# Shekhale/gbnns_dim_red

Hardware: AMD Instinct MI355X
Metric: queries/sec @ recall@1>=0.95, SIFT1M 128->32 (higher is better)
Workload: dtype f32

## Files before the change

### gbnns_dim_red_amd/csrc/walk_hot.hip

```cpp
#include "launch_util.h"
#include "walk_lists.h"

#ifndef GBNNS_HOT1_LB
#define GBNNS_HOT1_LB (GBNNS_HOT1_QLDS ? 8 : 7)
#endif
namespace gbnns {

namespace {


__device__ __forceinline__ bool reg1_select_slow(RegList<1>& L, uint64_t mu, int& tsize, uint64_t* tie, uint32_t worst,
                                                 uint64_t lmask, int lane, uint32_t& node) {
    int best = -1;
    uint32_t hi_p = 0;
    if (mu) {
        hi_p = readlane_u32(L.hi[0], __ffsll((unsigned long long)mu) - 1);
        const uint64_t ms = __ballot(!(L.lo[0] & 1u) && L.hi[0] == hi_p) & lmask;
        if (ms) best = 63 - __clzll((long long)ms);
    }
    if (tsize > 0 && (best < 0 || hi_p == worst)) {
        uint32_t v = (lane < tsize) ? key_id(tie[lane]) + 1u : 0u;
        int w = lane;
        int lane_here = lane;
        asm volatile("" : "+v"(lane_here));
#pragma unroll
        for (int off = 32; off > 0; off >>= 1) {
            const int partner = (lane_here ^ off) << 2;
            const uint32_t ov = (uint32_t)__builtin_amdgcn_ds_bpermute(partner, (int)v);
            const int ow = __builtin_amdgcn_ds_bpermute(partner, w);
            if (ov > v) { v = ov; w = ow; }
        }
        v = (uint32_t)__builtin_amdgcn_readfirstlane((int)v);
        w = __builtin_amdgcn_readfirstlane(w);
        const uint32_t lid = (best >= 0) ? (readlane_u32(L.lo[0], best) >> 1) : 0u;
        if (best < 0 || v - 1u > lid) {
            node = v - 1u;
            if (lane == 0) tie[w] = tie[tsize - 1];
            tsize -= 1;
            wave_sync();
            return true;
        }
    }
    if (best < 0) return false;
    node = readlane_u32(L.lo[0], best) >> 1;
    if (lane == best) L.lo[0] |= 1u;
    return true;
}

template <int R>
__device__ __forceinline__ bool regN_select_slow(RegList<R>& L, int p1, int& tsize, uint64_t* tie, uint32_t worst, int ef,
                                                 int lane, uint32_t& node) {
    int best = -1;
    uint32_t hi_p = 0;
    if (p1 >= 0) {
        hi_p = L.hi_at(p1);
#pragma unroll
        for (int r = 0; r < R; ++r) {
            const uint64_t ms = __ballot(!(L.lo[r] & 1u) && L.hi[r] == hi_p) & RegList<R>::lane_mask(r, ef);
            if (ms) best = r * 64 + 63 - __clzll((long long)ms);
        }
    }
    if (tsize > 0 && (best < 0 || hi_p == worst)) {
        uint32_t v = (lane < tsize) ? key_id(tie[lane]) + 1u : 0u;
        int w = lane;
        int lane_here = lane;
        asm volatile("" : "+v"(lane_here));
#pragma unroll
        for (int off = 32; off > 0; off >>= 1) {
            const int partner = (lane_here ^ off) << 2;
            const uint32_t ov = (uint32_t)__builtin_amdgcn_ds_bpermute(partner, (int)v);
            const int ow = __builtin_amdgcn_ds_bpermute(partner, w);
            if (ov > v) { v = ov; w = ow; }
        }
        v = (uint32_t)__builtin_amdgcn_readfirstlane((int)v);
        w = __builtin_amdgcn_readfirstlane(w);
        const uint32_t lid = (best >= 0) ? (L.lo_at(best) >> 1) : 0u;
        if (best < 0 || v - 1u > lid) {
            node = v - 1u;
            if (lane == 0) tie[w] = tie[tsize - 1];
            tsize -= 1;
            wave_sync();
            return true;
        }
    }
    if (best < 0) return false;
    node = L.lo_at(best) >> 1;
    L.mark_expanded(best, lane);
    return true;
}

#define GBNNS_VS_ASM(T0, T1, T2, ADDR)                                                                                                   \
        "s_bfe_u32 %[mulc], %[shr], 0x50008\n\t"                                    \
        "s_lshl_b32 %[mulc], 0x9E3779B1, %[mulc]\n\t"                                                                  \
        "v_mul_lo_u32 " T0 ", %[id], %[mulc]\n\t"                                                                       \
        "s_and_b32 exec_lo, exec_lo, 0x55555555\n\t"                                                                   \
        "s_and_b32 exec_hi, exec_hi, 0x55555555\n\t"                                                                   \
        "s_mov_b64 %[fresh], 0\n\t"                                                                                    \
        "s_cmp_lg_u32 %[shr], 0\n\t"                                                                                   \
        "v_mul_hi_u32 " T1 ", " T0 ", %[nb]\n\t"                                                                         \
        "v_lshl_add_u32 " ADDR ", " T1 ", 4, %[basev]\n\t"                                                               \
        "s_cbranch_scc1 4f\n"                                                                                          \
        "1:\n\t"                                                                                                       \
        "ds_read_b128 v[60:63], " ADDR "\n\t"                                                                           \
        "s_waitcnt lgkmcnt(0)\n\t"                                                                                     \
        "v_bfe_u32 v56, v60, 0, 24\n\t"                                                                    \
        "v_alignbit_b32 v57, v61, v60, 24\n\t"                            \
        "v_alignbit_b32 v58, v62, v61, 16\n\t"                                               \
        "v_lshrrev_b32 v59, 8, v62\n\t"                                                      \
        "v_bfe_u32 " T1 ", v63, 0, 24\n\t"                                                   \
        "v_bfe_u32 v57, v57, 0, 24\n\t"                                                                                \
        "v_bfe_u32 v58, v58, 0, 24\n\t"                                                                                \
        "v_xor_b32 v56, v56, %[id]\n\t"                                                                                \
        "v_xor_b32 v57, v57, %[id]\n\t"                                                                                \
        "v_xor_b32 v58, v58, %[id]\n\t"                                                                                \
        "v_xor_b32 v59, v59, %[id]\n\t"                                                                                \
        "v_xor_b32 " T1 ", " T1 ", %[id]\n\t"                                                                            \
        "v_min3_u32 v56, v56, v57, v58\n\t"                                                                            \
        "v_min3_u32 v56, v56, v59, " T1 "\n\t"                                           \
        "v_lshrrev_b32 " T1 ", 24, v63\n\t"                                                       \
        "v_cmp_ne_u32 vcc, 0, v56\n\t"                                                                                 \
        "s_and_b64 exec, exec, vcc\n\t"                                        \
        "s_cbranch_execz 9f\n\t"                                                                                       \
        "s_mov_b64 %[act], exec\n\t"                                                                                   \
        "v_cmp_gt_u32 vcc, 5, " T1 "\n\t"                                                                               \
        "s_and_b64 exec, exec, vcc\n\t"                                      \
        "s_cbranch_execz 3f\n\t"                                                                                       \
        "v_mov_b32 " T1 ", 0x1000000\n\t"                                                                               \
        "ds_add_rtn_u32 " T0 ", " ADDR ", " T1 " offset:12\n\t"                                   \
        "v_lshrrev_b32 " T2 ", 8, %[id]\n\t"                                                                            \
        "s_waitcnt lgkmcnt(0)\n\t"                                                                                     \
        "v_lshrrev_b32 " T0 ", 24, " T0 "\n\t"                                                                           \
        "v_cmp_gt_u32 vcc, 5, " T0 "\n\t"                                                                               \
        "s_and_b64 exec, exec, vcc\n\t"                                         \
        "s_cbranch_execz 3f\n\t"                                                                                       \
        "v_mad_u32_u24 " T0 ", " T0 ", 3, " ADDR "\n\t"                                     \
        "ds_write_b8 " T0 ", %[id]\n\t"                                                                                 \
        "ds_write_b8 " T0 ", " T2 " offset:1\n\t"                                                                        \
        "ds_write_b8_d16_hi " T0 ", %[id] offset:2\n\t"                                                                 \
        "s_or_b64 %[fresh], %[fresh], exec\n\t"                                                                        \
        "s_andn2_b64 %[act], %[act], exec\n"                                                                           \
        "3:\n\t"                                                                                                       \
        "s_mov_b64 exec, %[act]\n\t"                                    \
        "s_cbranch_execz 9f\n\t"                                                                                       \
        "v_add_u32 " ADDR ", 16, " ADDR "\n\t"                                                                           \
        "v_cmp_eq_u32 vcc, %[end], " ADDR "\n\t"                                                                        \
        "v_cndmask_b32 " ADDR ", " ADDR ", %[basev], vcc\n\t"                                                            \
        "s_branch 1b\n"                                                                                                \
        "4:\n\t"                                                                          \
        "s_lshl_b32 %[mulc], %[nb], 4\n\t"                                                                             \
        "v_mul_lo_u32 " T0 ", " T0 ", %[nb]\n\t"                               \
        "v_lshrrev_b32 " T0 ", %[shr], " T0 "\n\t"                                                           \
        "v_lshl_or_b32 " T2 ", " T0 ", 16, " T0 "\n"                          \
        "5:\n\t"                                                                                                       \
        "ds_read_b128 v[60:63], " ADDR "\n\t"                                                                           \
        "s_waitcnt lgkmcnt(0)\n\t"                                                                                     \
        "v_xor_b32 v56, v60, " T2 "\n\t"                                                                                \
        "v_xor_b32 v57, v61, " T2 "\n\t"                                                                                \
        "v_xor_b32 v58, v62, " T2 "\n\t"                                                                                \
        "v_xor_b32 v59, v63, " T2 "\n\t"                                                                                \
        "v_pk_min_u16 v56, v56, v57\n\t"                                                                               \
        "v_pk_min_u16 v58, v58, v59\n\t"                                                                               \
        "v_bfe_u32 " T1 ", v63, 16, 12\n\t"                                                       \
        "v_pk_min_u16 v56, v56, v58\n\t"                                                                               \
        "v_mad_u32_u16 v56, v56, v56, 0 op_sel:[0,1,0,0]\n\t"   \
        "v_cmp_ne_u32 vcc, 0, v56\n\t"                                                                                 \
        "s_and_b64 exec, exec, vcc\n\t"                                                                                \
        "s_cbranch_execz 9f\n\t"                                                                                       \
        "s_mov_b64 %[act], exec\n\t"                                                                                   \
        "v_cmp_gt_u32 vcc, 7, " T1 "\n\t"                                                                               \
        "s_and_b64 exec, exec, vcc\n\t"                                                                                \
        "s_cbranch_execz 6f\n\t"                                                                                       \
        "v_mov_b32 " T1 ", 0x10000\n\t"                                                                                 \
        "ds_add_rtn_u32 " T0 ", " ADDR ", " T1 " offset:12\n\t"                                                           \
        "s_waitcnt lgkmcnt(0)\n\t"                                                                                     \
        "v_bfe_u32 " T0 ", " T0 ", 16, 12\n\t"                                                                           \
        "v_cmp_gt_u32 vcc, 7, " T0 "\n\t"                                                                               \
        "s_and_b64 exec, exec, vcc\n\t"                                                                                \
        "s_cbranch_execz 6f\n\t"                                                                                       \
        "v_lshl_add_u32 " T0 ", " T0 ", 1, " ADDR "\n\t"                                                                  \
        "ds_write_b16 " T0 ", " T2 "\n\t"                                                                                \
        "s_or_b64 %[fresh], %[fresh], exec\n\t"                                                                        \
        "s_andn2_b64 %[act], %[act], exec\n"                                                                           \
        "6:\n\t"                                                                                                       \
        "s_mov_b64 exec, %[act]\n\t"                                                                                   \
        "s_cbranch_execz 9f\n\t"                                                                                       \
        "v_and_b32 " T0 ", 7, " T2 "\n\t"                         \
        "v_lshl_add_u32 " T0 ", " T0 ", 4, 16\n\t"                \
        "v_add_u32 " ADDR ", " ADDR ", " T0 "\n\t"                                                                        \
        "s_bfe_u32 vcc_lo, %[shr], 0x10010\n\t"                 \
        "s_lshl_b32 vcc_lo, 0x10001000, vcc_lo\n\t"                                                                    \
        "v_add_u32 " T2 ", vcc_lo, " T2 "\n\t"                                          \
        "v_cmp_le_u32 vcc, %[end], " ADDR "\n\t"                                                                        \
        "v_subrev_u32 " T0 ", %[mulc], " ADDR "\n\t"                       \
        "v_cndmask_b32 " ADDR ", " ADDR ", " T0 ", vcc\n\t"                                                               \
        "s_and_b32 vcc_lo, %[shr], 0xF0000000\n\t"            \
        "v_cmp_gt_u32 vcc, vcc_lo, " T2 "\n\t"                    \
        "s_andn2_b64 %[act], exec, vcc\n\t"                     \
        "s_lshl_b64 %[act], %[act], 1\n\t"                                                                             \
        "s_or_b64 %[fresh], %[fresh], %[act]\n\t"                                                                      \
        "s_and_b64 exec, exec, vcc\n\t"                                                                                \
        "s_cbranch_execnz 5b\n"                                                                                        \
        "9:\n\t"

#define GBNNS_L2_DIST_ASM(Q0A, Q0B, Q1A, Q1B, Q2A, Q2B, Q3A, Q3B, W1, W2, W3)                                                     \
        "s_waitcnt vmcnt(3)\n\t"                                \
        "v_pk_add_f32 v[40:41], v[40:41], " Q0A " neg_lo:[0,1] neg_hi:[0,1]\n\t"                                        \
        "v_pk_add_f32 v[42:43], v[42:43], " Q0B " neg_lo:[0,1] neg_hi:[0,1]\n\t"                                        \
        "v_pk_mul_f32 v[40:41], v[40:41], v[40:41]\n\t"                                                                \
        "v_pk_mul_f32 v[42:43], v[42:43], v[42:43]\n\t"                                                                \
        W1                                                                                                             \
        "v_pk_add_f32 v[44:45], v[44:45], " Q1A " neg_lo:[0,1] neg_hi:[0,1]\n\t"                                        \
        "v_pk_add_f32 v[46:47], v[46:47], " Q1B " neg_lo:[0,1] neg_hi:[0,1]\n\t"                                        \
        "v_pk_mul_f32 v[44:45], v[44:45], v[44:45]\n\t"                                                                \
        "v_pk_mul_f32 v[46:47], v[46:47], v[46:47]\n\t"                                                                \
        W2                                                                                                             \
        "v_pk_add_f32 v[48:49], v[48:49], " Q2A " neg_lo:[0,1] neg_hi:[0,1]\n\t"                                        \
        "v_pk_add_f32 v[50:51], v[50:51], " Q2B " neg_lo:[0,1] neg_hi:[0,1]\n\t"                                        \
        "v_pk_mul_f32 v[48:49], v[48:49], v[48:49]\n\t"                                                                \
        "v_pk_mul_f32 v[50:51], v[50:51], v[50:51]\n\t"                                                                \
        W3                                                                                                             \
        "v_pk_add_f32 v[52:53], v[52:53], " Q3A " neg_lo:[0,1] neg_hi:[0,1]\n\t"                                        \
        "v_pk_add_f32 v[54:55], v[54:55], " Q3B " neg_lo:[0,1] neg_hi:[0,1]\n\t"                                        \
        "v_pk_mul_f32 v[52:53], v[52:53], v[52:53]\n\t"                                                                \
        "v_pk_mul_f32 v[54:55], v[54:55], v[54:55]\n\t"                                                                \
        "v_pk_add_f32 v[60:61], v[40:41], v[44:45]\n\t"                                     \
        "v_pk_add_f32 v[62:63], v[42:43], v[46:47]\n\t"                                                                \
        "v_pk_add_f32 v[60:61], v[60:61], v[48:49]\n\t"                                                                \
        "v_pk_add_f32 v[62:63], v[62:63], v[50:51]\n\t"                                                                \
        "v_pk_add_f32 v[60:61], v[60:61], v[52:53]\n\t"                                                                \
        "v_pk_add_f32 v[62:63], v[62:63], v[54:55]\n\t"                                                                \
        "s_nop 1\n\t"                                                                                                  \
        "v_mov_b32_dpp v56, v60 quad_perm:[0,0,2,2] row_mask:0xf bank_mask:0xf\n\t"                                    \
        "v_mov_b32_dpp v57, v61 quad_perm:[0,0,2,2] row_mask:0xf bank_mask:0xf\n\t"                                    \
        "v_mov_b32_dpp v58, v62 quad_perm:[0,0,2,2] row_mask:0xf bank_mask:0xf\n\t"                                    \
        "v_mov_b32_dpp v59, v63 quad_perm:[0,0,2,2] row_mask:0xf bank_mask:0xf\n\t"                                    \
        "v_pk_add_f32 v[56:57], v[56:57], v[40:41]\n\t"                               \
        "v_pk_add_f32 v[58:59], v[58:59], v[42:43]\n\t"                                                                \
        "v_pk_add_f32 v[56:57], v[56:57], v[44:45]\n\t"                                                                \
        "v_pk_add_f32 v[58:59], v[58:59], v[46:47]\n\t"                                                                \
        "v_pk_add_f32 v[56:57], v[56:57], v[48:49]\n\t"                                                                \
        "v_pk_add_f32 v[58:59], v[58:59], v[50:51]\n\t"                                                                \
        "v_pk_add_f32 v[56:57], v[56:57], v[52:53]\n\t"                                                                \
        "v_pk_add_f32 v[58:59], v[58:59], v[54:55]\n\t"                                                                \
        "v_add_f32 %[key], v56, v57\n\t"                                                                               \
        "v_add_f32 %[key], %[key], v58\n\t"                                                                            \
        "v_add_f32 %[key], %[key], v59\n\t"                                                                            \
        "v_or_b32 %[key], 0x80000000, %[key]"

#define GBNNS_DOT_DIST_ASM(Q0A, Q0B, Q1A, Q1B, Q2A, Q2B, Q3A, Q3B, W1, W2, W3)                                                    \
        "s_waitcnt vmcnt(3)\n\t"                                                                                       \
        "v_pk_mul_f32 v[40:41], v[40:41], " Q0A "\n\t"                                                                 \
        "v_pk_mul_f32 v[42:43], v[42:43], " Q0B "\n\t"                                                                 \
        W1                                                                                                             \
        "v_pk_mul_f32 v[44:45], v[44:45], " Q1A "\n\t"                                                                 \
        "v_pk_mul_f32 v[46:47], v[46:47], " Q1B "\n\t"                                                                 \
        W2                                                                                                             \
        "v_pk_mul_f32 v[48:49], v[48:49], " Q2A "\n\t"                                                                 \
        "v_pk_mul_f32 v[50:51], v[50:51], " Q2B "\n\t"                                                                 \
        W3                                                                                                             \
        "v_pk_mul_f32 v[52:53], v[52:53], " Q3A "\n\t"                                                                 \
        "v_pk_mul_f32 v[54:55], v[54:55], " Q3B "\n\t"                                                                 \
        "v_mov_b32 v56, 0\n\t"                                     \
        "v_mov_b32 v57, 0\n\t"                                                                                         \
        "v_pk_add_f32 v[60:61], v[56:57], v[40:41]\n\t"           \
        "v_pk_add_f32 v[62:63], v[56:57], v[42:43]\n\t"                                                                \
        "v_pk_add_f32 v[60:61], v[60:61], v[44:45]\n\t"                                                                \
        "v_pk_add_f32 v[62:63], v[62:63], v[46:47]\n\t"                                                                \
        "v_pk_add_f32 v[60:61], v[60:61], v[48:49]\n\t"                                                                \
        "v_pk_add_f32 v[62:63], v[62:63], v[50:51]\n\t"                                                                \
        "v_pk_add_f32 v[60:61], v[60:61], v[52:53]\n\t"                                                                \
        "v_pk_add_f32 v[62:63], v[62:63], v[54:55]\n\t"                                                                \
        "s_nop 1\n\t"                                                                                                  \
        "v_mov_b32_dpp v56, v60 quad_perm:[0,0,2,2] row_mask:0xf bank_mask:0xf\n\t"      \
        "v_mov_b32_dpp v57, v61 quad_perm:[0,0,2,2] row_mask:0xf bank_mask:0xf\n\t"                                    \
        "v_mov_b32_dpp v58, v62 quad_perm:[0,0,2,2] row_mask:0xf bank_mask:0xf\n\t"                                    \
        "v_mov_b32_dpp v59, v63 quad_perm:[0,0,2,2] row_mask:0xf bank_mask:0xf\n\t"                                    \
        "v_pk_add_f32 v[56:57], v[60:61], v[56:57]\n\t"                             \
        "v_pk_add_f32 v[58:59], v[62:63], v[58:59]\n\t"                                                                \
        "v_add_f32 %[key], v56, v57\n\t"                                                    \
        "v_add_f32 v60, v58, v59\n\t"                                               \
        "v_add_f32 %[key], %[key], v60\n\t"                                                                            \
        "v_xor_b32 %[key], 0x80000000, %[key]\n\t"                                       \
        "v_add_f32 %[key], 0, %[key]\n\t"                                                         \
        "v_ashrrev_i32 v60, 31, %[key]\n\t"                     \
        "v_or_b32 v60, 0x80000000, v60\n\t"                                                                            \
        "v_xor_b32 %[key], %[key], v60"

#define GBNNS_LOADS_SPEC(O1, O2, O3)                                    \
        "global_load_dwordx4 v[40:43], %[roff], %[db]\n\t"              \
        "global_load_dwordx4 v[44:47], %[roff], %[db] offset:" O1 "\n\t" \
        "global_load_dwordx4 v[48:51], %[roff], %[db] offset:" O2 "\n\t" \
        "global_load_dwordx4 v[52:55], %[roff], %[db] offset:" O3 "\n\t"
#define GBNNS_LOADS_TESTED(O1, O2, O3)                                                                                 \
        "s_lshr_b64 %[act], %[fresh], 1\n\t"                             \
        "s_or_b64 exec, %[act], %[fresh]\n\t"                                                                          \
        "s_and_b32 exec_lo, exec_lo, 0x55555555\n\t"                                     \
        "s_and_b32 exec_hi, exec_hi, 0x55555555\n\t"                                                                   \
        "s_lshl_b64 %[act], exec, 1\n\t"                                                                               \
        "s_or_b64 exec, exec, %[act]\n\t"                                              \
        "s_cbranch_execz 8f\n\t"                                                                                       \
        GBNNS_LOADS_SPEC(O1, O2, O3)                                                                                   \
        "s_mov_b64 exec, %[sv]\n\t"
#define GBNNS_LOADS_DYN_BEFORE(O1, O2, O3)      \
        "s_cmp_eq_u32 %[spec], 0\n\t"           \
        "s_cbranch_scc1 12f\n\t"                \
        GBNNS_LOADS_SPEC(O1, O2, O3)            \
        "12:\n\t"
#define GBNNS_LOADS_DYN_AFTER(O1, O2, O3)       \
        "s_cmp_lg_u32 %[spec], 0\n\t"           \
        "s_cbranch_scc0 10f\n\t"                \
        "s_mov_b64 exec, %[sv]\n\t"             \
        "s_branch 11f\n"                        \
        "10:\n\t"                               \
        GBNNS_LOADS_TESTED(O1, O2, O3)          \
        "11:\n\t"
#define GBNNS_HOT_END "\n8:\n\ts_mov_b64 exec, %[sv]"

#define GBNNS_HOT_CLOBBERS_40                                                                                           \
    "vcc", "scc", "memory", "v40", "v41", "v42", "v43", "v44", "v45", "v46", "v47", "v48", "v49", "v50", "v51", "v52", "v53", "v54",  \
        "v55", "v56", "v57", "v58", "v59", "v60", "v61", "v62", "v63"

template <int METRIC = 0, bool QLDS = false, bool SPEC = !QLDS, bool DYN = false, typename QP>
__device__ __forceinline__ uint32_t hot_expand(const char* db_base, uint32_t roff, uint32_t nb, uint64_t valid, uint32_t lds_base,
                                               uint32_t nbuckets, QP qh, uint32_t qaddr, uint64_t& claimed, uint32_t shr, uint64_t& overflowed,
                                               uint32_t spec = 0u) {
    const uint32_t end = lds_base + (nbuckets << 4);
    uint32_t basev = lds_base, key, mulc;
    uint64_t fresh, act, sv;
#define GBNNS_Q(T) [qa##T] "v"(f32x2{qh[T].x, qh[T].y}), [qb##T] "v"(f32x2{qh[T].z, qh[T].w})
#define GBNNS_HOT_OUT [fresh] "=&s"(fresh), [act] "=&s"(act), [sv] "=&s"(sv), [mulc] "=&s"(mulc), [key] "=&v"(key)
#define GBNNS_HOT_IN [id] "v"(nb), [valid] "s"(valid), [end] "s"(end), [basev] "v"(basev), [shr] "s"(shr), [nb] "s"(nbuckets), \
                     [roff] "v"(roff), [db] "s"(db_base)
#define GBNNS_HOT_IN_QREG GBNNS_HOT_IN, GBNNS_Q(0), GBNNS_Q(1), GBNNS_Q(2), GBNNS_Q(3)
#define GBNNS_HOT_IN_QLDS GBNNS_HOT_IN, [qaddr] "v"(qaddr)
#define GBNNS_HOT_IN_QLDS_DYN GBNNS_HOT_IN_QLDS, [spec] "s"(spec)
#define GBNNS_HOT_OUT_QREG GBNNS_HOT_OUT, [t0] "=&v"(t0), [t1] "=&v"(t1), [t2] "=&v"(t2), [addr] "=&v"(addr)
#define GBNNS_HOT_OUT_QLDS GBNNS_HOT_OUT
#define GBNNS_VS_QREG GBNNS_VS_ASM("%[t0]", "%[t1]", "%[t2]", "%[addr]")
#define GBNNS_VS_QLDS GBNNS_VS_ASM("v36", "v37", "v38", "v39")
#define GBNNS_CLOB_QREG GBNNS_HOT_CLOBBERS_40
#define GBNNS_CLOB_QLDS "v36", "v37", "v38", "v39", GBNNS_HOT_CLOBBERS_40
#define GBNNS_HOT_STMT(LOADS_BEFORE, VS, AFTER_VS, DIST, OUTS, OPS, CLOB)                      \
    asm volatile("s_mov_b64 %[sv], exec\n\t"                                                   \
                 "s_mov_b64 exec, %[valid]\n\t" LOADS_BEFORE VS AFTER_VS DIST GBNNS_HOT_END      \
                 : OUTS                                                                        \
                 : OPS                                                                         \
                 : CLOB)
#define GBNNS_RESTORE_EXEC "s_mov_b64 exec, %[sv]\n\t"
#define GBNNS_L2_QREG                                                                                                          \
    GBNNS_L2_DIST_ASM("%[qa0]", "%[qb0]", "%[qa1]", "%[qb1]", "%[qa2]", "%[qb2]", "%[qa3]", "%[qb3]", "s_waitcnt vmcnt(2)\n\t", \
                      "s_waitcnt vmcnt(1)\n\t", "s_waitcnt vmcnt(0)\n\t")
#define GBNNS_L2_QLDS                                                                                                          \
    "ds_read_b128 v[36:39], %[qaddr]\n\t"                       \
    "ds_read_b128 v[56:59], %[qaddr] offset:16\n\t"           \
    "ds_read_b128 v[60:63], %[qaddr] offset:32\n\t"                                                                           \
    "s_waitcnt lgkmcnt(2)\n\t"                                                                                                \
    GBNNS_L2_DIST_ASM("v[36:37]", "v[38:39]", "v[56:57]", "v[58:59]", "v[60:61]", "v[62:63]", "v[36:37]", "v[38:39]",          \
                      "ds_read_b128 v[36:39], %[qaddr] offset:48\n\ts_waitcnt vmcnt(2) lgkmcnt(2)\n\t",                        \
                      "s_waitcnt vmcnt(1) lgkmcnt(1)\n\t", "s_waitcnt vmcnt(0) lgkmcnt(0)\n\t")
#define GBNNS_DOT_QREG                                                                                                          \
    GBNNS_DOT_DIST_ASM("%[qa0]", "%[qb0]", "%[qa1]", "%[qb1]", "%[qa2]", "%[qb2]", "%[qa3]", "%[qb3]", "s_waitcnt vmcnt(2)\n\t", \
                       "s_waitcnt vmcnt(1)\n\t", "s_waitcnt vmcnt(0)\n\t")
#define GBNNS_DOT_QLDS                                                                                                         \
    "ds_read_b128 v[36:39], %[qaddr]\n\t"                                                                                     \
    "ds_read_b128 v[56:59], %[qaddr] offset:32\n\t"                                                                           \
    "ds_read_b128 v[60:63], %[qaddr] offset:64\n\t"                                                                           \
    "s_waitcnt lgkmcnt(2)\n\t"                                                                                                \
    GBNNS_DOT_DIST_ASM("v[36:37]", "v[38:39]", "v[56:57]", "v[58:59]", "v[60:61]", "v[62:63]", "v[36:37]", "v[38:39]",         \
                       "ds_read_b128 v[36:39], %[qaddr] offset:96\n\ts_waitcnt vmcnt(2) lgkmcnt(2)\n\t",                       \
                       "s_waitcnt vmcnt(1) lgkmcnt(1)\n\t", "s_waitcnt vmcnt(0) lgkmcnt(0)\n\t")
    uint32_t t0, t1, t2, addr;
    (void)t0; (void)t1; (void)t2; (void)addr;
    if constexpr (DYN) {
        static_assert(!DYN || QLDS, "the dynamic order exists for the query-in-LDS instances");
        if constexpr (METRIC == 0) GBNNS_HOT_STMT(GBNNS_LOADS_DYN_BEFORE("16", "32", "48"), GBNNS_VS_QLDS, GBNNS_LOADS_DYN_AFTER("16", "32", "48"), GBNNS_L2_QLDS, GBNNS_HOT_OUT_QLDS, GBNNS_HOT_IN_QLDS_DYN, GBNNS_CLOB_QLDS);
        else GBNNS_HOT_STMT(GBNNS_LOADS_DYN_BEFORE("32", "64", "96"), GBNNS_VS_QLDS, GBNNS_LOADS_DYN_AFTER("32", "64", "96"), GBNNS_DOT_QLDS, GBNNS_HOT_OUT_QLDS, GBNNS_HOT_IN_QLDS_DYN, GBNNS_CLOB_QLDS);
    } else if constexpr (METRIC == 0) {
        if constexpr (!QLDS && SPEC) GBNNS_HOT_STMT(GBNNS_LOADS_SPEC("16", "32", "48"), GBNNS_VS_QREG, GBNNS_RESTORE_EXEC, GBNNS_L2_QREG, GBNNS_HOT_OUT_QREG, GBNNS_HOT_IN_QREG, GBNNS_CLOB_QREG);
        else if constexpr (!QLDS) GBNNS_HOT_STMT("", GBNNS_VS_QREG, GBNNS_LOADS_TESTED("16", "32", "48"), GBNNS_L2_QREG, GBNNS_HOT_OUT_QREG, GBNNS_HOT_IN_QREG, GBNNS_CLOB_QREG);
        else if constexpr (SPEC) GBNNS_HOT_STMT(GBNNS_LOADS_SPEC("16", "32", "48"), GBNNS_VS_QLDS, GBNNS_RESTORE_EXEC, GBNNS_L2_QLDS, GBNNS_HOT_OUT_QLDS, GBNNS_HOT_IN_QLDS, GBNNS_CLOB_QLDS);
        else GBNNS_HOT_STMT("", GBNNS_VS_QLDS, GBNNS_LOADS_TESTED("16", "32", "48"), GBNNS_L2_QLDS, GBNNS_HOT_OUT_QLDS, GBNNS_HOT_IN_QLDS, GBNNS_CLOB_QLDS);
    } else {
        if constexpr (!QLDS && SPEC) GBNNS_HOT_STMT(GBNNS_LOADS_SPEC("32", "64", "96"), GBNNS_VS_QREG, GBNNS_RESTORE_EXEC, GBNNS_DOT_QREG, GBNNS_HOT_OUT_QREG, GBNNS_HOT_IN_QREG, GBNNS_CLOB_QREG);
        else if constexpr (!QLDS) GBNNS_HOT_STMT("", GBNNS_VS_QREG, GBNNS_LOADS_TESTED("32", "64", "96"), GBNNS_DOT_QREG, GBNNS_HOT_OUT_QREG, GBNNS_HOT_IN_QREG, GBNNS_CLOB_QREG);
        else if constexpr (SPEC) GBNNS_HOT_STMT(GBNNS_LOADS_SPEC("32", "64", "96"), GBNNS_VS_QLDS, GBNNS_RESTORE_EXEC, GBNNS_DOT_QLDS, GBNNS_HOT_OUT_QLDS, GBNNS_HOT_IN_QLDS, GBNNS_CLOB_QLDS);
        else GBNNS_HOT_STMT("", GBNNS_VS_QLDS, GBNNS_LOADS_TESTED("32", "64", "96"), GBNNS_DOT_QLDS, GBNNS_HOT_OUT_QLDS, GBNNS_HOT_IN_QLDS, GBNNS_CLOB_QLDS);
    }
#undef GBNNS_HOT_STMT
#undef GBNNS_HOT_IN_QREG
#undef GBNNS_HOT_IN_QLDS
#undef GBNNS_HOT_IN_QLDS_DYN
#undef GBNNS_CLOB_QLDS
#undef GBNNS_CLOB_QREG
#undef GBNNS_VS_QLDS
#undef GBNNS_VS_QREG
#undef GBNNS_HOT_OUT_QLDS
#undef GBNNS_HOT_OUT_QREG
#undef GBNNS_Q
#undef GBNNS_HOT_OUT
#undef GBNNS_HOT_IN
    claimed = fresh & 0x5555555555555555ull;
    overflowed = fresh & 0xAAAAAAAAAAAAAAAAull;
    return key;
}

template <int R, bool WIDE = false, int METRIC = 0, bool SPEC1 = GBNNS_HOT1_SPEC != 0>
__device__ __forceinline__ void walk_hot_one(const WalkParams& p, uint32_t qi, unsigned char* smem) {
    const int lane = lane_id();
    const uint32_t slot = (uint32_t)lane >> 1, half = (uint32_t)lane & 1u;
    const int ef = p.ef;
#ifdef GBNNS_LIFE_STAMPS
    const unsigned long long life0 = __builtin_amdgcn_s_memrealtime();
#endif
    constexpr bool QLDS = R == 1 && GBNNS_HOT1_QLDS, SPEC = R == 1 ? SPEC1 : true;
    uint64_t* tie = reinterpret_cast<uint64_t*>(smem);
    uint64_t* stage = tie + kRegTieCap;
    float* qf = reinterpret_cast<float*>(QLDS ? stage + reg_stage_slots(R) : stage);
    uint32_t* hash = reinterpret_cast<uint32_t*>(stage + reg_stage_slots(R)) + (QLDS ? 32 : 0);
    const float4* qs = reinterpret_cast<const float4*>(qf);
    const uint32_t cap = p.hash_cap;
    const uint32_t hash_lds = (uint32_t)(size_t)((__attribute__((address_space(3))) unsigned char*)reinterpret_cast<unsigned char*>(hash));

    const uint32_t vs_shr = p.vs_shr;
    const uint32_t nbuckets = vs_shr ? cap / 7u - kStashBuckets : cap / 5u;
    if (vs_shr) quotient_table_init(hash, nbuckets, lane);
    else packed_table_init(hash, nbuckets, 0u, lane);
    if (lane < 32) qf[lane] = p.q[(size_t)qi * p.qstride + lane];
    wave_sync();
    RowRegs<4> qreg;
    if constexpr (!QLDS) {
#pragma unroll
        for (int t = 0; t < 4; ++t) qreg.v[t] = METRIC == 0 ? qs[4 * half + t] : qs[2 * t + half];
    }
    const uint32_t qaddr = (uint32_t)(size_t)((__attribute__((address_space(3))) unsigned char*)reinterpret_cast<unsigned char*>(qf)) +
                           half * (METRIC == 0 ? 64u : 16u);

    RegList<R> L;
    L.clear();
    int size = 1, tsize = 0, hops = 0, dist_calc = 1, edges = 0;
    uint32_t worst;
    const uint32_t entry = p.entries ? p.entries[qi] : 0u;
    if (entry >= p.n) { write_bad_entry(p, qi, lane); return; }
    {
        const float d0 = walk_dist<METRIC, 8>(qs, row_ptr<true>(p.db, entry, 32u), 32u);
        worst = fkey(d0);
        if (lane == 0) {
            L.hi[0] = worst;
            L.lo[0] = entry << 1;
            if (vs_shr) quotient_table_put_first(hash, nbuckets, entry, vs_shr);
            else packed_table_put_first(hash, nbuckets, entry);
        }
        wave_sync();
    }

    const uint64_t lmask = RegList<R>::lane_mask(0, ef);
    const uint32_t ell_row_bytes = p.ell_stride * 4u;
    const bool slot_ok = slot < p.ell_stride;
    const uint32_t slot_off = slot_ok ? slot * 4u : 0u;
    const bool slotw_ok = WIDE && slot + 32u < p.ell_stride;
    const uint32_t slotw_off = slotw_ok ? (slot + 32u) * 4u : 0u;
    const char* ell_base = reinterpret_cast<const char*>(p.ell);
    const char* db_base = reinterpret_cast<const char*>(p.db);
    const uint32_t dc_limit = p.hash_limit >= 32u ? p.hash_limit - 32u : 0u;
    bool handed_over = false;
    const uint32_t spec_tail = (uint32_t)__builtin_amdgcn_readfirstlane((int)(blockIdx.x >= p.spec_from));
    uint32_t pf_node = kInvalidId, pf_val = kInvalidId;
    uint32_t pf2_node = kInvalidId, pf2_val = kInvalidId;
    uint32_t pf_valw = kInvalidId, pf2_valw = kInvalidId;
#ifdef GBNNS_LIFE_STAMPS
    const unsigned long long life1 = __builtin_amdgcn_s_memrealtime();
#endif

    while (true) {
        uint32_t node, pred, ok, h2;
        if constexpr (R == 1) {
            uint64_t fm;
            uint32_t t0, q1, q2, h1;
            asm volatile(
                "v_and_b32 %[t0], 1, %[lo]\n\t"
                "v_cmp_eq_u32 vcc, 0, %[t0]\n\t"
                "s_and_b64 %[fm], vcc, %[lmask]\n\t"
                "s_cmp_eq_u32 %[tsize], 0\n\t"
                "s_cselect_b64 %[fm], %[fm], 0\n\t"
                "s_ff1_i32_b64 %[q1], %[fm]\n\t"
                "s_bitset0_b64 %[fm], %[q1]\n\t"
                "s_ff1_i32_b64 %[q2], %[fm]\n\t"
                "v_readlane_b32 %[h1], %[hi], %[q1]\n\t"
                "v_readlane_b32 %[node], %[lo], %[q1]\n\t"
                "v_readlane_b32 %[h2], %[hi], %[q2]\n\t"
                "v_readlane_b32 %[pred], %[lo], %[q2]\n\t"
                "s_lshr_b32 %[node], %[node], 1\n\t"
                "s_lshr_b32 %[pred], %[pred], 1\n\t"
                "s_cmp_lg_u32 %[h1], %[h2]\n\t"
                "s_cselect_b32 %[ok], 1, 0\n\t"
                "s_cmp_lt_i32 %[q2], 0\n\t"
                "s_cselect_b32 %[ok], 1, %[ok]\n\t"
                "s_cselect_b32 %[pred], -1, %[pred]\n\t"
                "s_cselect_b32 %[h2], -1, %[h2]\n\t"
                "s_cmp_lt_i32 %[q1], 0\n\t"
                "s_cselect_b32 %[ok], 0, %[ok]\n\t"
                "s_cmp_lg_u32 %[ok], 0\n\t"
                "s_cselect_b32 %[q1], %[q1], -1\n\t"
                "v_cmp_eq_u32 vcc, %[q1], %[lane]\n\t"
                "v_cndmask_b32 %[t0], 0, 1, vcc\n\t"
                "v_or_b32 %[lo], %[lo], %[t0]"
                : [lo] "+v"(L.lo[0]), [fm] "=&s"(fm), [t0] "=&v"(t0), [q1] "=&s"(q1), [q2] "=&s"(q2), [h1] "=&s"(h1),
                  [h2] "=&s"(h2), [node] "=&s"(node), [pred] "=&s"(pred), [ok] "=&s"(ok)
                : [hi] "v"(L.hi[0]), [lmask] "s"(lmask), [tsize] "s"(tsize), [lane] "v"(lane)
                : "vcc", "scc");
            if (__builtin_expect(ok == 0, 0)) {
                const uint64_t mu = __ballot(!(L.lo[0] & 1u)) & lmask;
                if (!reg1_select_slow(L, mu, tsize, tie, worst, lmask, lane, node)) break;
                pred = kInvalidId;
                h2 = 0xFFFFFFFFu;
            }
        } else {
            int p1 = -1, p2 = -1;
#pragma unroll
            for (int r = 0; r < R; ++r) {
                uint64_t mm = __ballot(!(L.lo[r] & 1u)) & RegList<R>::lane_mask(r, ef);
                if (p1 < 0 && mm) {
                    p1 = r * 64 + __ffsll((unsigned long long)mm) - 1;
                    mm &= mm - 1;
                }
                if (p1 >= 0 && p2 < 0 && mm) p2 = r * 64 + __ffsll((unsigned long long)mm) - 1;
            }
            ok = 0; node = 0; pred = kInvalidId; h2 = 0xFFFFFFFFu;
            if (p1 >= 0 && tsize == 0) {
                if (p2 >= 0) {
                    const uint32_t hp2 = L.hi_at(p2);
                    if (L.hi_at(p1) != hp2) {
                        ok = 1;
                        node = L.lo_at(p1) >> 1;
                        pred = L.lo_at(p2) >> 1;
                        h2 = hp2;
                        L.mark_expanded(p1, lane);
                    }
                } else {
                    ok = 1;
                    node = L.lo_at(p1) >> 1;
                    L.mark_expanded(p1, lane);
                }
            }
            if (__builtin_expect(ok == 0, 0)) {
                if (!regN_select_slow<R>(L, p1, tsize, tie, worst, ef, lane, node)) break;
            }
        }

        uint32_t nb, nbw = kInvalidId;
        if (node == pf_node) {
            nb = pf_val;
            if constexpr (WIDE) nbw = pf_valw;
        } else if (node == pf2_node) {
            nb = pf2_val;
            if constexpr (WIDE) nbw = pf2_valw;
        } else {
            nb = *reinterpret_cast<const uint32_t*>(ell_base + node * ell_row_bytes + slot_off);
            if constexpr (WIDE) nbw = *reinterpret_cast<const uint32_t*>(ell_base + node * ell_row_bytes + slotw_off);
        }
        nb = slot_ok ? nb : kInvalidId;
        if constexpr (WIDE) nbw = slotw_ok ? nbw : kInvalidId;
        pf2_node = kInvalidId;
        const uint64_t mv0 = __ballot(nb != kInvalidId);
        const uint64_t mv1 = WIDE ? __ballot(nbw != kInvalidId) : 0ull;
        pf_node = pred;
        if (pred != kInvalidId) {
            pf_val = *reinterpret_cast<const uint32_t*>(ell_base + pred * ell_row_bytes + slot_off);
            if constexpr (WIDE) pf_valw = *reinterpret_cast<const uint32_t*>(ell_base + pred * ell_row_bytes + slotw_off);
        }
        auto expand_pass = [&](const uint32_t nb, const uint64_t mv) -> bool {
            if (__builtin_expect(mv == 0, 0)) return true;
            if (__builtin_expect((uint32_t)dist_calc > dc_limit, 0)) return false;
            edges += __popcll(mv & 0x5555555555555555ull);
            uint64_t mclaimed, movf;
            const uint32_t kd = hot_expand<METRIC, QLDS, SPEC, (QLDS && !SPEC)>(db_base, (nb << 7) + half * (METRIC == 0 ? 64u : 16u), nb, mv, hash_lds, nbuckets, qreg.v, qaddr, mclaimed, vs_shr, movf, spec_tail);
            if (__builtin_expect(movf != 0, 0)) {
                if (!stash_claim(hash_lds, nbuckets, movf >> 1, nb, mclaimed, lane)) return false;
            }
            const uint64_t mfresh = mclaimed << 1;
            const uint32_t dk = __builtin_amdgcn_inverse_ballot_w64(mfresh) ? kd : 0xFFFFFFFFu;
            dist_calc += __popcll(mfresh);
            uint64_t m = size < ef ? mfresh : __ballot(dk < worst);
            if (m != 0) {
                auto prefetch2 = [&](const uint32_t dmin, const uint64_t me) {
                    if (dmin < h2 && me != 0 && (me & (me - 1)) == 0) {
                        pf2_node = readlane_u32(nb, __ffsll((unsigned long long)me) - 1);
                        pf2_val = *reinterpret_cast<const uint32_t*>(ell_base + pf2_node * ell_row_bytes + slot_off);
                        if constexpr (WIDE) {
                            pf2_valw = *reinterpret_cast<const uint32_t*>(ell_base + pf2_node * ell_row_bytes + slotw_off);
                            h2 = dmin;
                        }
                    }
                };
                bool merged = false;
                if constexpr (R == 1 && GBNNS_HOT1_PF2_IN_MERGE) {
                    if ((m & (m - 1)) != 0) {
                        merged = reg_merge_cb<true>(m, __builtin_amdgcn_inverse_ballot_w64(m), dk, nb, L, size, worst, tsize, stage, ef, lane,
                                                    [&](const uint32_t dmin) { if (dmin < h2) prefetch2(dmin, __ballot(dk == dmin) & m); });
                    } else {
                        prefetch2(readlane_u32(dk, __ffsll((unsigned long long)m) - 1), m);
                    }
                } else {
                    uint32_t x = dk;
                    x = min(x, (uint32_t)__builtin_amdgcn_update_dpp((int)x, (int)x, 0xB1, 0xf, 0xf, false));
                    x = min(x, (uint32_t)__builtin_amdgcn_update_dpp((int)x, (int)x, 0x4E, 0xf, 0xf, false));
                    x = min(x, (uint32_t)__builtin_amdgcn_update_dpp((int)x, (int)x, 0x141, 0xf, 0xf, false));
                    x = min(x, (uint32_t)__builtin_amdgcn_update_dpp((int)x, (int)x, 0x140, 0xf, 0xf, false));
                    const uint32_t dmin = min(min(readlane_u32(x, 0), readlane_u32(x, 16)), min(readlane_u32(x, 32), readlane_u32(x, 48)));
                    if (dmin < h2) prefetch2(dmin, __ballot(dk == dmin) & m);
                    if ((m & (m - 1)) != 0) {
                        if constexpr (R == 1) merged = reg_merge(m, __builtin_amdgcn_inverse_ballot_w64(m), dk, nb, L, size, worst, tsize, stage, ef, lane);
                        else merged = reg_merge_multi<R>(m, __builtin_amdgcn_inverse_ballot_w64(m), dk, nb, L, size, worst, tsize, stage, ef, lane);
                    }
                }
                if (!merged) {
                    do {
                        const int l = __ffsll((unsigned long long)m) - 1;
                        m &= m - 1;
                        if (!reg_offer<R>(readlane_u32(dk, l), readlane_u32(nb, l) << 1, L, size, worst, tsize, tie, ef, lane)) return false;
                    } while (m);
                }
            }
            return true;
        };
        if (!expand_pass(nb, mv0)) { handed_over = true; break; }
        if constexpr (WIDE) {
            if (!expand_pass(nbw, mv1)) { handed_over = true; break; }
        }
        hops += 1;
    }

    if (handed_over) {
        if (lane == 0) {
            const uint32_t s = atomicAdd(p.ovf_count, 1u);
            p.ovf_list[s] = qi;
        }
        return;
    }
#ifdef GBNNS_LIFE_STAMPS
    const unsigned long long life2 = __builtin_amdgcn_s_memrealtime();
#endif
    reg_write_results<R>(p, qi, L, size, hops, dist_calc, edges, lane);
    if (p.rr_db) {
        const int kept = size < p.k ? size : p.k;
        fused_rerank(p, qi, kept, smem, lane, [&](int rank) { return reg_id_at_rank<R>(L, rank); });
    }
#ifdef GBNNS_LIFE_STAMPS
    {
        asm volatile("s_waitcnt vmcnt(0) lgkmcnt(0)" ::: "memory");
        const unsigned long long life3 = __builtin_amdgcn_s_memrealtime();
        if (lane == 0 && p.stamps) {
            atomicAdd(p.stamps + 0, life1 - life0); atomicAdd(p.stamps + 1, life2 - life1); atomicAdd(p.stamps + 2, life3 - life2);
            atomicAdd(p.stamps + 3, 1ull);
            atomicMax(p.stamps + 4, life3 - life0);
            atomicMax(p.stamps + 5, (1ull << 62) - life0); atomicMax(p.stamps + 6, life0); atomicMax(p.stamps + 7, life3);
        }
    }
#endif
}

template <bool WIDE = false, int METRIC = 0>
__device__ __forceinline__ void walk_hot_big(const WalkParams& p, uint32_t qi, unsigned char* smem) {
    const int lane = lane_id();
#ifdef GBNNS_STAMPS
    unsigned long long seg[8] = {0, 0, 0, 0, 0, 0, 0, 0};
    unsigned st_pf1 = 0, st_pf2 = 0;
    STAMP(t_begin)
    unsigned long long t_prev = t_begin;
#endif
    const uint32_t slot = (uint32_t)lane >> 1, half = (uint32_t)lane & 1u;
    const int ef = p.ef;
    BigList B;
    B.init(smem, ef);
    float* qf = reinterpret_cast<float*>(B.stage);
    unsigned char* hash_bytes = smem + big_list_fixed_bytes(ef);
    uint32_t* hash = reinterpret_cast<uint32_t*>(hash_bytes);
    const float4* qs = reinterpret_cast<const float4*>(qf);
    const uint32_t cap = p.hash_cap;
    const uint32_t hash_lds = (uint32_t)(size_t)((__attribute__((address_space(3))) unsigned char*)reinterpret_cast<unsigned char*>(hash));
    const uint32_t vs_shr = p.vs_shr;
    const uint32_t nbuckets = vs_shr ? cap / 7u - kStashBuckets : cap / 5u;
    if (vs_shr) quotient_table_init(hash, nbuckets, lane);
    else packed_table_init(hash, nbuckets, 0u, lane);
    if (lane < 32) qf[lane] = p.q[(size_t)qi * p.qstride + lane];
    wave_sync();
    RowRegs<4> qreg;
#pragma unroll
    for (int t = 0; t < 4; ++t) qreg.v[t] = METRIC == 0 ? qs[4 * half + t] : qs[2 * t + half];

    int hops = 0, dist_calc = 1, edges = 0;
    const uint32_t entry = (uint32_t)__builtin_amdgcn_readfirstlane((int)(p.entries ? p.entries[qi] : 0u));
    if (entry >= p.n) { write_bad_entry(p, qi, lane); return; }
    {
        const float d0 = walk_dist<METRIC, 8>(qs, row_ptr<true>(p.db, entry, 32u), 32u);
        B.worst = B.fworst = (uint32_t)__builtin_amdgcn_readfirstlane((int)fkey(d0));
        if (lane == 0) {
            B.F.hi[0] = B.worst;
            B.F.lo[0] = entry << 1;
            if (vs_shr) quotient_table_put_first(hash, nbuckets, entry, vs_shr);
            else packed_table_put_first(hash, nbuckets, entry);
        }
        wave_sync();
    }

    const uint32_t ell_row_bytes = p.ell_stride * 4u;
    const bool slot_ok = slot < p.ell_stride;
    const uint32_t slot_off = slot_ok ? slot * 4u : 0u;
    const bool slotw_ok = WIDE && slot + 32u < p.ell_stride;
    const uint32_t slotw_off = slotw_ok ? (slot + 32u) * 4u : 0u;
    const char* ell_base = reinterpret_cast<const char*>(p.ell);
    const char* db_base = reinterpret_cast<const char*>(p.db);
    const uint32_t dc_limit = p.hash_limit >= 32u ? p.hash_limit - 32u : 0u;
    bool handed_over = false;
    uint32_t pf_node = kInvalidId, pf_val = kInvalidId, pf2_node = kInvalidId, pf2_val = kInvalidId;
    uint32_t pf_valw = kInvalidId, pf2_valw = kInvalidId;

    while (true) {
        uint32_t node, pred, h2;
        STAMP(t0)
        STAMP_ADD(7, t_prev, t0)
        if (!B.select(node, pred, h2, lane)) break;
        STAMP(t1)
        STAMP_ADD(0, t0, t1)

        uint32_t nb, nbw = kInvalidId;
#ifdef GBNNS_STAMPS
        if (node == pf_node) st_pf1 += 1;
        else if (node == pf2_node) st_pf2 += 1;
#endif
        if (node == pf_node) {
            nb = pf_val;
            if constexpr (WIDE) nbw = pf_valw;
        } else if (node == pf2_node) {
            nb = pf2_val;
            if constexpr (WIDE) nbw = pf2_valw;
        } else {
            nb = *reinterpret_cast<const uint32_t*>(ell_base + node * ell_row_bytes + slot_off);
            if constexpr (WIDE) nbw = *reinterpret_cast<const uint32_t*>(ell_base + node * ell_row_bytes + slotw_off);
        }
        nb = slot_ok ? nb : kInvalidId;
        if constexpr (WIDE) nbw = slotw_ok ? nbw : kInvalidId;
        pf2_node = kInvalidId;
        const uint64_t mv0 = __ballot(nb != kInvalidId);
        const uint64_t mv1 = WIDE ? __ballot(nbw != kInvalidId) : 0ull;
        STAMP(t2)
        STAMP_ADD(1, t1, t2)
        pf_node = pred;
        if (pred != kInvalidId) {
            pf_val = *reinterpret_cast<const uint32_t*>(ell_base + pred * ell_row_bytes + slot_off);
            if constexpr (WIDE) pf_valw = *reinterpret_cast<const uint32_t*>(ell_base + pred * ell_row_bytes + slotw_off);
        }
        auto expand_pass = [&](const uint32_t nb, const uint64_t mv) -> bool {
            if (__builtin_expect(mv == 0, 0)) return true;
            if (__builtin_expect((uint32_t)dist_calc > dc_limit, 0)) return false;
            edges += __popcll(mv & 0x5555555555555555ull);
            STAMP(t3)
            STAMP_ADD(2, t2, t3)
            uint64_t mclaimed, movf;
            const uint32_t kd = hot_expand<METRIC, false, true>(db_base, (nb << 7) + half * (METRIC == 0 ? 64u : 16u), nb, mv, hash_lds, nbuckets, qreg.v, 0u, mclaimed, vs_shr, movf);
            if (__builtin_expect(movf != 0, 0)) {
                if (!stash_claim(hash_lds, nbuckets, movf >> 1, nb, mclaimed, lane)) return false;
            }
            const uint64_t mfresh = mclaimed << 1;
            const uint32_t dk = __builtin_amdgcn_inverse_ballot_w64(mfresh) ? kd : 0xFFFFFFFFu;
            dist_calc += __popcll(mfresh);
            const uint64_t m = (B.l + B.f < ef) ? mfresh : __ballot(dk < B.worst);
            STAMP(t5)
            STAMP_ADD(4, t3, t5)
            if (m != 0) {
                {
                    uint32_t x = dk;
                    x = min(x, (uint32_t)__builtin_amdgcn_update_dpp((int)x, (int)x, 0xB1, 0xf, 0xf, false));
                    x = min(x, (uint32_t)__builtin_amdgcn_update_dpp((int)x, (int)x, 0x4E, 0xf, 0xf, false));
                    x = min(x, (uint32_t)__builtin_amdgcn_update_dpp((int)x, (int)x, 0x141, 0xf, 0xf, false));
                    x = min(x, (uint32_t)__builtin_amdgcn_update_dpp((int)x, (int)x, 0x140, 0xf, 0xf, false));
                    const uint32_t dmin = min(min(readlane_u32(x, 0), readlane_u32(x, 16)), min(readlane_u32(x, 32), readlane_u32(x, 48)));
                    if (dmin < h2) {
                        const uint64_t me = __ballot(dk == dmin) & m;
                        if (me != 0 && (me & (me - 1)) == 0) {
                            pf2_node = readlane_u32(nb, __ffsll((unsigned long long)me) - 1);
                            pf2_val = *reinterpret_cast<const uint32_t*>(ell_base + pf2_node * ell_row_bytes + slot_off);
                            if constexpr (WIDE) {
                                pf2_valw = *reinterpret_cast<const uint32_t*>(ell_base + pf2_node * ell_row_bytes + slotw_off);
                                h2 = dmin;
                            }
                        }
                    }
                }
                if (!B.insert(m, dk, nb, lane)) return false;
            }
            STAMP(t6)
            STAMP_ADD(5, t5, t6)
#ifdef GBNNS_STAMPS
            t_prev = t6;
#endif
            return true;
        };
        if (!expand_pass(nb, mv0)) { handed_over = true; break; }
        if constexpr (WIDE) {
            if (!expand_pass(nbw, mv1)) { handed_over = true; break; }
        }
        hops += 1;
    }

#ifdef GBNNS_STAMPS
    {
        STAMP(t_end)
        seg[6] = t_end - t_begin;
        if (lane == 0 && p.stamps) {
            for (int i = 0; i < 7; ++i) atomicAdd(p.stamps + i, seg[i]);
            atomicAdd(p.stamps + 30, seg[7]);
            atomicAdd(p.stamps + 21, B.st_flush); atomicAdd(p.stamps + 22, B.st_refresh); atomicAdd(p.stamps + 23, B.st_evict);
            atomicAdd(p.stamps + 24, (unsigned long long)B.st_nflush); atomicAdd(p.stamps + 25, (unsigned long long)B.st_nrefresh);
            atomicAdd(p.stamps + 26, (unsigned long long)B.st_nbase); atomicAdd(p.stamps + 27, (unsigned long long)B.st_nseq);
            atomicAdd(p.stamps + 28, (unsigned long long)B.st_ninsert); atomicAdd(p.stamps + 29, (unsigned long long)B.st_slow);
            atomicAdd(p.stamps + 7, (unsigned long long)st_pf1); atomicAdd(p.stamps + 31, (unsigned long long)st_pf2);
        }
    }
#endif
    if (handed_over) {
        if (lane == 0) {
            const uint32_t s = atomicAdd(p.ovf_count, 1u);
            p.ovf_list[s] = qi;
        }
        return;
    }
    B.finish(p, qi, hops, dist_calc, edges, hash_bytes, lane);
}

__global__ __launch_bounds__(64) void walk_hot2_kernel(WalkParams p) {
    extern __shared__ __attribute__((aligned(16))) unsigned char smem[];
    walk_hot_one<2>(p, walk_query_of(p, blockIdx.x), smem);
}

__global__ __launch_bounds__(64) void walk_hot_big_kernel(WalkParams p) {
    extern __shared__ __attribute__((aligned(16))) unsigned char smem[];
    walk_hot_big(p, walk_query_of(p, blockIdx.x), smem);
}

__global__ __launch_bounds__(64, GBNNS_HOT1_LB) void walk_hot_kernel(WalkParams p) {
    extern __shared__ __attribute__((aligned(16))) unsigned char smem[];
#ifdef GBNNS_HOT1_CAP6
    asm volatile("" ::: "s96");
#endif
    walk_hot_one<1>(p, walk_query_of(p, blockIdx.x), smem);
}

__global__ __launch_bounds__(64, GBNNS_HOT1_LB) void walk_hot_spec_kernel(WalkParams p) {
    extern __shared__ __attribute__((aligned(16))) unsigned char smem[];
    walk_hot_one<1, false, 0, true>(p, walk_query_of(p, blockIdx.x), smem);
}

__global__ __launch_bounds__(64, GBNNS_HOT1_LB) void walk_hotw_kernel(WalkParams p) {
    extern __shared__ __attribute__((aligned(16))) unsigned char smem[];
    walk_hot_one<1, true>(p, walk_query_of(p, blockIdx.x), smem);
}

__global__ __launch_bounds__(64) void walk_hotw2_kernel(WalkParams p) {
    extern __shared__ __attribute__((aligned(16))) unsigned char smem[];
    walk_hot_one<2, true>(p, walk_query_of(p, blockIdx.x), smem);
}

__global__ __launch_bounds__(64) void walk_hotw_big_kernel(WalkParams p) {
    extern __shared__ __attribute__((aligned(16))) unsigned char smem[];
    walk_hot_big<true>(p, walk_query_of(p, blockIdx.x), smem);
}

template <int R, bool WIDE>
__global__ __launch_bounds__(64, R == 1 && GBNNS_HOT1_QLDS ? 8 : 1) void walk_hot_dot_kernel(WalkParams p) {
    extern __shared__ __attribute__((aligned(16))) unsigned char smem[];
    walk_hot_one<R, WIDE, 1>(p, walk_query_of(p, blockIdx.x), smem);
}

template <bool WIDE>
__global__ __launch_bounds__(64) void walk_hot_dot_big_kernel(WalkParams p) {
    extern __shared__ __attribute__((aligned(16))) unsigned char smem[];
    walk_hot_big<WIDE, 1>(p, walk_query_of(p, blockIdx.x), smem);
}

}

hipError_t launch_walk_hot(const WalkParams& p, int metric, hipStream_t s) {
    const size_t lds = walk_fast_lds_bytes(p, true);
    const bool wide = p.ell_stride > 32u;
    if (p.ef <= 64) {
        if (metric == 1) return wide ? launch_walk_k(walk_hot_dot_kernel<1, true>, p, false, lds, s) : launch_walk_k(walk_hot_dot_kernel<1, false>, p, false, lds, s);
        if (!wide && p.spec_rows && !GBNNS_HOT1_SPEC) return launch_walk_k(walk_hot_spec_kernel, p, false, lds, s);
        return wide ? launch_walk_k(walk_hotw_kernel, p, false, lds, s) : launch_walk_k(walk_hot_kernel, p, false, lds, s);
    }
    if (p.ef <= kHot2MaxEf) {
        if (metric == 1) return wide ? launch_walk_k(walk_hot_dot_kernel<2, true>, p, false, lds, s) : launch_walk_k(walk_hot_dot_kernel<2, false>, p, false, lds, s);
        return wide ? launch_walk_k(walk_hotw2_kernel, p, false, lds, s) : launch_walk_k(walk_hot2_kernel, p, false, lds, s);
    }
    if (metric == 1) return wide ? launch_walk_k(walk_hot_dot_big_kernel<true>, p, false, lds, s) : launch_walk_k(walk_hot_dot_big_kernel<false>, p, false, lds, s);
    return wide ? launch_walk_k(walk_hotw_big_kernel, p, false, lds, s) : launch_walk_k(walk_hot_big_kernel, p, false, lds, s);
}

}
```

### gbnns_dim_red_amd/csrc/walk_lists.h

```cpp
#pragma once

#include "walk_common.h"

namespace gbnns {

namespace {


__device__ __forceinline__ uint32_t writelane_u32(uint32_t vdst, uint32_t val, int l) {
    asm("s_mov_b32 m0, %2\n\tv_writelane_b32 %0, %1, m0" : "+v"(vdst) : "s"(val), "s"(l) : "m0");
    return vdst;
}
__device__ __forceinline__ uint64_t clear_bit64(uint64_t m, int bit) {
    asm("s_bitset0_b64 %0, %1" : "+s"(m) : "s"(bit));
    return m;
}

#ifndef GBNNS_HOT1_QLDS
#define GBNNS_HOT1_QLDS 1
#endif
#ifndef GBNNS_HOT1_SPEC
#define GBNNS_HOT1_SPEC 0
#endif
#ifndef GBNNS_WIDE_VGPRS
#define GBNNS_WIDE_VGPRS 80
#endif
#ifndef GBNNS_HOT1_PF2_IN_MERGE
#define GBNNS_HOT1_PF2_IN_MERGE 0
#endif
constexpr int kRegTieCap = 16;
constexpr int kRegListMaxEf = 1024;

__device__ __forceinline__ uint32_t dpp_wave_shr1(uint32_t v) {
    return (uint32_t)__builtin_amdgcn_update_dpp((int)v, (int)v, 0x138, 0xf, 0xf, false);
}
__device__ __forceinline__ uint32_t readlane_u32(uint32_t v, int l) {
    return (uint32_t)__builtin_amdgcn_readlane((int)v, l);
}

#ifdef GBNNS_STAMPS
#define STAMP(var)                                                                        \
    unsigned long long var;                                                               \
    __builtin_amdgcn_sched_barrier(0);                                                    \
    asm volatile("s_memtime %0\n\ts_waitcnt lgkmcnt(0)" : "=s"(var)::"memory");           \
    __builtin_amdgcn_sched_barrier(0);
#define STAMP_ADD(i, a, b) seg[i] += (b) - (a);
#else
#define STAMP(var)
#define STAMP_ADD(i, a, b)
#endif

template <int STEPS>
struct RowRegs {
    float4 v[STEPS > 0 ? STEPS : 1];
};

template <int STEPS>
__device__ __forceinline__ void load_row(RowRegs<STEPS>& r, const float* row) {
    const float4* r4 = reinterpret_cast<const float4*>(row);
#pragma unroll
    for (int t = 0; t < STEPS; ++t) r.v[t] = r4[t];
}

template <int STEPS, typename QP>
__device__ __forceinline__ float l2_from_regs(const RowRegs<STEPS>& r, QP qs) {
    float s0 = 0.f, s1 = 0.f, s2 = 0.f, s3 = 0.f;
#pragma unroll
    for (int t = 0; t < STEPS; ++t) {
        const float4 bv = qs[t];
        float e;
        e = r.v[t].x - bv.x; s0 = s0 + e * e;  e = r.v[t].y - bv.y; s1 = s1 + e * e;
        e = r.v[t].z - bv.z; s2 = s2 + e * e;  e = r.v[t].w - bv.w; s3 = s3 + e * e;
    }
    return ((s0 + s1) + s2) + s3;
}

typedef float f32x2 __attribute__((ext_vector_type(2)));

#define GBNNS_L2_STEP(T)                                                        \
    "v_pk_add_f32 %[ta], %[a" #T "], %[qa" #T "] neg_lo:[0,1] neg_hi:[0,1]\n\t" \
    "v_pk_add_f32 %[tb], %[b" #T "], %[qb" #T "] neg_lo:[0,1] neg_hi:[0,1]\n\t" \
    "v_pk_mul_f32 %[ta], %[ta], %[ta]\n\t"                                     \
    "v_pk_mul_f32 %[tb], %[tb], %[tb]\n\t"                                     \
    "v_pk_add_f32 %[sa], %[sa], %[ta]\n\t"                                     \
    "v_pk_add_f32 %[sb], %[sb], %[tb]\n\t"

template <typename QP>
__device__ __forceinline__ float l2_from_regs8(const RowRegs<8>& r, QP qs) {
    f32x2 sa, sb, ta, tb;
#define GBNNS_PAIRS(T)                                                                          \
    [a##T] "v"(f32x2{r.v[T].x, r.v[T].y}), [b##T] "v"(f32x2{r.v[T].z, r.v[T].w}),                \
    [qa##T] "v"(f32x2{qs[T].x, qs[T].y}), [qb##T] "v"(f32x2{qs[T].z, qs[T].w})
    asm("v_pk_add_f32 %[ta], %[a0], %[qa0] neg_lo:[0,1] neg_hi:[0,1]\n\t"
        "v_pk_add_f32 %[tb], %[b0], %[qb0] neg_lo:[0,1] neg_hi:[0,1]\n\t"
        "v_pk_mul_f32 %[sa], %[ta], %[ta]\n\t"
        "v_pk_mul_f32 %[sb], %[tb], %[tb]\n\t"
        GBNNS_L2_STEP(1) GBNNS_L2_STEP(2) GBNNS_L2_STEP(3)
        : [sa] "=&v"(sa), [sb] "=&v"(sb), [ta] "=&v"(ta), [tb] "=&v"(tb)
        : GBNNS_PAIRS(0), GBNNS_PAIRS(1), GBNNS_PAIRS(2), GBNNS_PAIRS(3));
    asm(GBNNS_L2_STEP(4) GBNNS_L2_STEP(5) GBNNS_L2_STEP(6) GBNNS_L2_STEP(7)
        : [sa] "+v"(sa), [sb] "+v"(sb), [ta] "=&v"(ta), [tb] "=&v"(tb)
        : GBNNS_PAIRS(4), GBNNS_PAIRS(5), GBNNS_PAIRS(6), GBNNS_PAIRS(7));
#undef GBNNS_PAIRS
    return ((sa.x + sa.y) + sb.x) + sb.y;
}
#undef GBNNS_L2_STEP

#define GBNNS_P_SUB(T)                                                                  \
    "v_pk_add_f32 %[pa" #T "], %[a" #T "], %[qa" #T "] neg_lo:[0,1] neg_hi:[0,1]\n\t" \
    "v_pk_add_f32 %[pb" #T "], %[b" #T "], %[qb" #T "] neg_lo:[0,1] neg_hi:[0,1]\n\t"
#define GBNNS_P_MUL(T)                                           \
    "v_pk_mul_f32 %[pa" #T "], %[pa" #T "], %[pa" #T "]\n\t" \
    "v_pk_mul_f32 %[pb" #T "], %[pb" #T "], %[pb" #T "]\n\t"
#define GBNNS_P_ACC(T)                                         \
    "v_pk_add_f32 v[64:65], v[64:65], %[pa" #T "]\n\t"      \
    "v_pk_add_f32 v[66:67], v[66:67], %[pb" #T "]\n\t"
template <typename QP>
__device__ __forceinline__ float l2_pair_from_regs(const RowRegs<4>& r, QP qh) {
    f32x2 pa0, pb0, pa1, pb1, pa2, pb2, pa3, pb3;
    float d;
#define GBNNS_Q(T)                                                                               \
    [a##T] "v"(f32x2{r.v[T].x, r.v[T].y}), [b##T] "v"(f32x2{r.v[T].z, r.v[T].w}),                \
    [qa##T] "v"(f32x2{qh[T].x, qh[T].y}), [qb##T] "v"(f32x2{qh[T].z, qh[T].w})
    asm(GBNNS_P_SUB(0) GBNNS_P_SUB(1) GBNNS_P_MUL(0) GBNNS_P_MUL(1) GBNNS_P_SUB(2) GBNNS_P_SUB(3) GBNNS_P_MUL(2) GBNNS_P_MUL(3)
        "v_pk_add_f32 v[68:69], %[pa0], %[pa1]\n\t"
        "v_pk_add_f32 v[70:71], %[pb0], %[pb1]\n\t"
        "v_pk_add_f32 v[68:69], v[68:69], %[pa2]\n\t"
        "v_pk_add_f32 v[70:71], v[70:71], %[pb2]\n\t"
        "v_pk_add_f32 v[68:69], v[68:69], %[pa3]\n\t"
        "v_pk_add_f32 v[70:71], v[70:71], %[pb3]\n\t"
        "s_nop 1\n\t"
        "v_mov_b32_dpp v64, v68 quad_perm:[0,0,2,2] row_mask:0xf bank_mask:0xf\n\t"
        "v_mov_b32_dpp v65, v69 quad_perm:[0,0,2,2] row_mask:0xf bank_mask:0xf\n\t"
        "v_mov_b32_dpp v66, v70 quad_perm:[0,0,2,2] row_mask:0xf bank_mask:0xf\n\t"
        "v_mov_b32_dpp v67, v71 quad_perm:[0,0,2,2] row_mask:0xf bank_mask:0xf\n\t"
        GBNNS_P_ACC(0) GBNNS_P_ACC(1) GBNNS_P_ACC(2) GBNNS_P_ACC(3)
        "v_add_f32 %[d], v64, v65\n\t"
        "v_add_f32 %[d], %[d], v66\n\t"
        "v_add_f32 %[d], %[d], v67"
        : [d] "=&v"(d), [pa0] "=&v"(pa0), [pb0] "=&v"(pb0), [pa1] "=&v"(pa1), [pb1] "=&v"(pb1), [pa2] "=&v"(pa2),
          [pb2] "=&v"(pb2), [pa3] "=&v"(pa3), [pb3] "=&v"(pb3)
        : GBNNS_Q(0), GBNNS_Q(1), GBNNS_Q(2), GBNNS_Q(3)
        : "v64", "v65", "v66", "v67", "v68", "v69", "v70", "v71");
#undef GBNNS_Q
    return d;
}
#undef GBNNS_P_SUB
#undef GBNNS_P_MUL
#undef GBNNS_P_ACC

__device__ __forceinline__ float dpp_from_even(float x) {
    return __int_as_float(__builtin_amdgcn_update_dpp(0, __float_as_int(x), 0xA0, 0xf, 0xf, false));
}
template <int H, typename QP>
__device__ __forceinline__ float l2_pair_from_regs_wide(const RowRegs<H>& r, QP qh) {
    f32x2 ea[H], eb[H];
#pragma unroll
    for (int t = 0; t < H; ++t) {
        const float4 a = r.v[t], b = qh[t];
        const f32x2 da = f32x2{a.x, a.y} - f32x2{b.x, b.y}, db = f32x2{a.z, a.w} - f32x2{b.z, b.w};
        ea[t] = da * da;
        eb[t] = db * db;
    }
    f32x2 sa = ea[0], sb = eb[0];
#pragma unroll
    for (int t = 1; t < H; ++t) { sa = sa + ea[t]; sb = sb + eb[t]; }
    auto from_even = [](float v) {
        return __int_as_float(__builtin_amdgcn_update_dpp(0, __float_as_int(v), 0xA0, 0xf, 0xf, false));
    };
    f32x2 ta = f32x2{from_even(sa.x), from_even(sa.y)}, tb = f32x2{from_even(sb.x), from_even(sb.y)};
#pragma unroll
    for (int t = 0; t < H; ++t) { ta = ta + ea[t]; tb = tb + eb[t]; }
    return ((ta.x + ta.y) + tb.x) + tb.y;
}

template <typename QP>
__device__ __forceinline__ float dot_pair_from_regs(const RowRegs<4>& r, QP qh) {
    float c0 = 0.f, c1 = 0.f, c2 = 0.f, c3 = 0.f;
#pragma unroll
    for (int t = 0; t < 4; ++t) {
        c0 = c0 + r.v[t].x * qh[t].x; c1 = c1 + r.v[t].y * qh[t].y;
        c2 = c2 + r.v[t].z * qh[t].z; c3 = c3 + r.v[t].w * qh[t].w;
    }
    const float m0 = c0 + dpp_from_even(c0), m1 = c1 + dpp_from_even(c1);
    const float m2 = c2 + dpp_from_even(c2), m3 = c3 + dpp_from_even(c3);
    return -((m0 + m1) + (m2 + m3));
}
__device__ __forceinline__ void load_row_alt(RowRegs<4>& r, const float* row) {
    const float4* r4 = reinterpret_cast<const float4*>(row);
#pragma unroll
    for (int t = 0; t < 4; ++t) r.v[t] = r4[2 * t];
}

template <bool OFF32>
__device__ __forceinline__ const float* row_ptr(const float* base, uint32_t id, uint32_t stride_floats) {
    if constexpr (OFF32) {
        const uint32_t off = id * (stride_floats * 4u);
        return reinterpret_cast<const float*>(reinterpret_cast<const char*>(base) + off);
    } else {
        return base + (size_t)id * stride_floats;
    }
}

template <bool OFF32>
__device__ __forceinline__ float l2_quad_rows(uint64_t mfresh, uint32_t nb, const float* db, uint32_t dstride, uint32_t dim, const float* qf, int lane) {
    float out = 0.f;
    const uint32_t steps = dim >> 2;
    const int g = lane >> 2, j = lane & 3;
    const float* q = qf + j;
    uint64_t m = mfresh;
    while (m) {
        uint64_t round = 0ull, mm = m;
        int src = 0;
#pragma unroll
        for (int i = 0; i < 16; ++i) {
            const int pos = mm ? __ffsll((unsigned long long)mm) - 1 : 0;
            round |= mm ? (1ull << pos) : 0ull;
            mm &= mm - 1ull;
            src = (g == i) ? pos : src;
        }
        const int nrows = __popcll(round);
        uint32_t id = (uint32_t)__builtin_amdgcn_ds_bpermute(src << 2, (int)nb);
        id = g < nrows ? id : 0u;
        const float* row = row_ptr<OFF32>(db, id, dstride) + j;
        float sum = 0.f;
        uint32_t t = 0;
        for (; t + 16 <= steps; t += 16) {
            float r[16];
#pragma unroll
            for (int k = 0; k < 16; ++k) r[k] = row[4u * (t + k)];
#pragma unroll
            for (int k = 0; k < 16; ++k) {
                const float e = q[4u * (t + k)] - r[k];
                sum = sum + e * e;
            }
        }
        if (t < steps) {
            float r[16], qv[16];
#pragma unroll
            for (int k = 0; k < 16; ++k) {
                const bool in = t + k < steps;
                r[k] = in ? row[4u * (t + k)] : 0.f;
                qv[k] = in ? q[4u * (t + k)] : 0.f;
            }
#pragma unroll
            for (int k = 0; k < 16; ++k) {
                const float e = qv[k] - r[k];
                sum = sum + e * e;
            }
        }
        const int si = __float_as_int(sum);
        const float s0 = __int_as_float(__builtin_amdgcn_update_dpp(0, si, 0x00, 0xf, 0xf, false));
        const float s1 = __int_as_float(__builtin_amdgcn_update_dpp(0, si, 0x55, 0xf, 0xf, false));
        const float s2 = __int_as_float(__builtin_amdgcn_update_dpp(0, si, 0xAA, 0xf, 0xf, false));
        const float s3 = __int_as_float(__builtin_amdgcn_update_dpp(0, si, 0xFF, 0xf, 0xf, false));
        const float d = ((s0 + s1) + s2) + s3;
        const int rank = __popcll(round & ((1ull << lane) - 1ull));
        const float dv = __int_as_float(__builtin_amdgcn_ds_bpermute(rank << 4, __float_as_int(d)));
        out = ((round >> lane) & 1ull) ? dv : out;
        m &= ~round;
    }
    return out;
}

template <int R>
struct RegList {
    uint32_t lo[R], hi[R];

    __device__ __forceinline__ void clear() {
#pragma unroll
        for (int r = 0; r < R; ++r) lo[r] = hi[r] = 0xFFFFFFFFu;
    }
    __device__ __forceinline__ uint32_t lo_at(int rank) const {
        uint32_t v = readlane_u32(lo[0], rank & 63);
#pragma unroll
        for (int r = 1; r < R; ++r) {
            const uint32_t t = readlane_u32(lo[r], rank & 63);
            if ((rank >> 6) == r) v = t;
        }
        return v;
    }
    __device__ __forceinline__ uint32_t hi_at(int rank) const {
        uint32_t v = readlane_u32(hi[0], rank & 63);
#pragma unroll
        for (int r = 1; r < R; ++r) {
            const uint32_t t = readlane_u32(hi[r], rank & 63);
            if ((rank >> 6) == r) v = t;
        }
        return v;
    }
    __device__ __forceinline__ void mark_expanded(int rank, int lane) {
#pragma unroll
        for (int r = 0; r < R; ++r)
            if ((rank >> 6) == r && lane == (rank & 63)) lo[r] |= 1u;
    }
    __device__ __forceinline__ static uint64_t lane_mask(int r, int ef) {
        const int left = ef - r * 64;
        return left >= 64 ? ~0ull : (left <= 0 ? 0ull : ((1ull << left) - 1ull));
    }
};

template <int R>
__device__ __forceinline__ bool reg_offer(uint32_t dl, uint32_t nlo, RegList<R>& L, int& size, uint32_t& worst,
                                          int& tsize, uint64_t* tie, int ef, int lane) {
    const bool full = size >= ef;
    if (full && !(dl < worst)) return true;
    const uint64_t nk = ((uint64_t)dl << 32) | nlo;
    const uint32_t ev_lo = L.lo_at(ef - 1);
    uint32_t c_lt = 1u, c_lo = 0u, c_hi = 0u;
#pragma unroll
    for (int r = 0; r < R; ++r) {
        const uint64_t key = ((uint64_t)L.hi[r] << 32) | L.lo[r];
        const bool lt = key < nk;
        const uint32_t lt_i = lt ? 1u : 0u;
        const uint32_t lt_left = (uint32_t)__builtin_amdgcn_update_dpp((int)c_lt, (int)lt_i, 0x138, 0xf, 0xf, false);
        const uint32_t slo = (uint32_t)__builtin_amdgcn_update_dpp((int)c_lo, (int)L.lo[r], 0x138, 0xf, 0xf, false);
        const uint32_t shi = (uint32_t)__builtin_amdgcn_update_dpp((int)c_hi, (int)L.hi[r], 0x138, 0xf, 0xf, false);
        if (r + 1 < R) {
            c_lt = readlane_u32(lt_i, 63);
            c_lo = readlane_u32(L.lo[r], 63);
            c_hi = readlane_u32(L.hi[r], 63);
        }
        if (!lt) {
            L.lo[r] = lt_left ? nlo : slo;
            L.hi[r] = lt_left ? dl : shi;
        }
    }
    if (!full) {
        size += 1;
        worst = L.hi_at(size - 1);
        return true;
    }
    const uint32_t nw = L.hi_at(ef - 1);
    if (nw != worst) {
        tsize = 0;
    } else if (!(ev_lo & 1u)) {
        if (tsize >= kRegTieCap) return false;
        if (lane == 0) tie[tsize] = ((uint64_t)worst << 32) | ev_lo;
        tsize += 1;
        wave_sync();
    }
    worst = nw;
    return true;
}

#ifdef GBNNS_MERGE_S98
#define GBNNS_MERGE_SLO "s98"
#define GBNNS_MERGE_SHI "s99"
#define GBNNS_MERGE_SPAIR "s[98:99]"
#else
#define GBNNS_MERGE_SLO "s46"
#define GBNNS_MERGE_SHI "s47"
#define GBNNS_MERGE_SPAIR "s[46:47]"
#endif
constexpr int kRegStageSlots = 66;

template <bool WANT_MIN, typename AfterRanks>
__device__ __forceinline__ bool reg_merge_cb(uint64_t m, bool is_surv, uint32_t dk, uint32_t nb, RegList<1>& L, int& size,
                                             uint32_t& worst, int& tsize, uint64_t* stage, int ef, int lane, AfterRanks&& after_ranks) {
    const int ns = __popcll(m);
    const uint64_t key = ((uint64_t)L.hi[0] << 32) | L.lo[0];
    const uint32_t slo = nb << 1;
    const uint64_t skey = ((uint64_t)dk << 32) | slo;
    const bool is_entry = lane < size;
    uint32_t shift, rank, below, sl_, t_, smin = 0xFFFFFFFFu;
    uint64_t ma, mb, mm = m;
#define GBNNS_RANK_LOOP(MIN_STEP)                                                                                       \
    asm volatile(                                                                                                      \
        "v_mov_b32 %[shift], 0\n\t"                                                                                    \
        "v_mov_b32 %[rank], 0\n\t"                                                                                     \
        "v_mov_b32 %[below], 0\n"                                                                                      \
        "1:\n\t"                                                                                                       \
        "s_ff1_i32_b64 %[sl], %[mm]\n\t"                                                                               \
        "v_readlane_b32 " GBNNS_MERGE_SHI ", %[dk], %[sl]\n\t"                                                                         \
        "v_readlane_b32 " GBNNS_MERGE_SLO ", %[slo], %[sl]\n\t"                                                                        \
        "s_bitset0_b64 %[mm], %[sl]\n\t"                                                                               \
        "s_mov_b32 m0, %[sl]\n\t"                                                                                      \
        "v_cmp_gt_u64_e64 %[ma], %[key], " GBNNS_MERGE_SPAIR "\n\t"                                                                 \
        "v_cmp_gt_u64_e64 %[mb], %[skey], " GBNNS_MERGE_SPAIR "\n\t" MIN_STEP                                                       \
        "s_bcnt0_i32_b64 %[t], %[ma]\n\t"                                                                              \
        "v_addc_co_u32_e64 %[shift], vcc, 0, %[shift], %[ma]\n\t"                                                      \
        "v_addc_co_u32_e64 %[rank], vcc, 0, %[rank], %[mb]\n\t"                                                        \
        "v_writelane_b32 %[below], %[t], m0\n\t"                                                                       \
        "s_cmp_lg_u64 %[mm], 0\n\t"                                                                                    \
        "s_cbranch_scc1 1b"                                                                                            \
        : [shift] "=&v"(shift), [rank] "=&v"(rank), [below] "=&v"(below), [sl] "=&s"(sl_), [t] "=&s"(t_), [ma] "=&s"(ma), \
          [mb] "=&s"(mb), [mm] "+s"(mm), [smin] "+s"(smin)                                                              \
        : [dk] "v"(dk), [slo] "v"(slo), [key] "v"(key), [skey] "v"(skey)                                                \
        : "vcc", "scc", "m0", GBNNS_MERGE_SLO, GBNNS_MERGE_SHI)
    if constexpr (WANT_MIN) {
        GBNNS_RANK_LOOP("s_min_u32 %[smin], %[smin], " GBNNS_MERGE_SHI "\n\t");
        after_ranks(smin);
    } else {
        GBNNS_RANK_LOOP("");
    }
#undef GBNNS_RANK_LOOP
    const int dst_e = lane + (int)shift, dst_s = (int)(rank + below);
    const int total = size + ns;
    const int new_size = total < ef ? total : ef;
    if (is_entry && dst_e <= ef) stage[dst_e] = key;
    if (is_surv && dst_s <= ef) stage[dst_s] = skey;
    wave_sync();
    const uint64_t nkey = lane < new_size ? stage[lane] : ~0ull;
    const uint32_t nw = readlane_u32((uint32_t)(nkey >> 32), new_size - 1);
    if (total > ef) {
        const uint32_t first_dropped = (uint32_t)__builtin_amdgcn_readfirstlane((int)(stage[ef] >> 32));
        if (first_dropped == nw) return false;
        tsize = 0;
    }
    L.lo[0] = (uint32_t)nkey;
    L.hi[0] = (uint32_t)(nkey >> 32);
    size = new_size;
    worst = nw;
    return true;
}

__device__ __forceinline__ bool reg_merge(uint64_t m, bool is_surv, uint32_t dk, uint32_t nb, RegList<1>& L, int& size,
                                          uint32_t& worst, int& tsize, uint64_t* stage, int ef, int lane) {
    return reg_merge_cb<false>(m, is_surv, dk, nb, L, size, worst, tsize, stage, ef, lane, [](uint32_t) {});
}

__device__ __forceinline__ constexpr int reg_stage_slots(int R) { return 64 * R + 2; }

template <int R>
__device__ __forceinline__ bool reg_merge_multi(uint64_t m, bool is_surv, uint32_t dk, uint32_t nb, RegList<R>& L, int& size,
                                                uint32_t& worst, int& tsize, uint64_t* stage, int ef, int lane) {
    const int ns = __popcll(m);
    uint64_t key[R];
#pragma unroll
    for (int r = 0; r < R; ++r) key[r] = ((uint64_t)L.hi[r] << 32) | L.lo[r];
    const uint32_t slo = nb << 1;
    const uint64_t skey = ((uint64_t)dk << 32) | slo;
    uint32_t shift[R];
#pragma unroll
    for (int r = 0; r < R; ++r) shift[r] = 0;
    uint32_t rank = 0, below = 0;
    uint64_t mm = m;
    do {
        const int sl = __ffsll((unsigned long long)mm) - 1;
        mm = clear_bit64(mm, sl);
        const uint64_t ks = ((uint64_t)readlane_u32(dk, sl) << 32) | readlane_u32(slo, sl);
        uint32_t cnt = 0;
#pragma unroll
        for (int r = 0; r < R; ++r) {
            const bool gt = key[r] > ks;
            shift[r] += gt ? 1u : 0u;
            cnt += (uint32_t)__popcll(~__ballot(gt));
        }
        rank += skey > ks ? 1u : 0u;
        below = writelane_u32(below, cnt, sl);
    } while (mm);
    const int total = size + ns;
    const int new_size = total < ef ? total : ef;
#pragma unroll
    for (int r = 0; r < R; ++r) {
        const int re = r * 64 + lane, dst = re + (int)shift[r];
        if (re < size && dst <= ef) stage[dst] = key[r];
    }
    {
        const int dst_s = (int)(rank + below);
        if (is_surv && dst_s <= ef) stage[dst_s] = skey;
    }
    wave_sync();
    uint32_t first_dropped = 0;
    if (total > ef) first_dropped = (uint32_t)__builtin_amdgcn_readfirstlane((int)(stage[ef] >> 32));
    uint32_t nlo[R], nhi[R], nw = 0;
#pragma unroll
    for (int r = 0; r < R; ++r) {
        const uint64_t v = (r * 64 + lane < new_size) ? stage[r * 64 + lane] : ~0ull;
        nlo[r] = (uint32_t)v;
        nhi[r] = (uint32_t)(v >> 32);
        const uint32_t t = readlane_u32(nhi[r], (new_size - 1) & 63);
        if (((new_size - 1) >> 6) == r) nw = t;
    }
    wave_sync();
    if (total > ef && first_dropped == nw) return false;
    if (total > ef) tsize = 0;
#pragma unroll
    for (int r = 0; r < R; ++r) {
        L.lo[r] = nlo[r];
        L.hi[r] = nhi[r];
    }
    size = new_size;
    worst = nw;
    return true;
}

template <int R>
__device__ __forceinline__ void reg_write_results(const WalkParams& p, uint32_t qi, const RegList<R>& L, int size, int hops,
                                                  int dist_calc, int edges, int lane) {
    const int kept = size < p.k ? size : p.k;
    const uint32_t kth = L.lo_at(kept > 0 ? kept - 1 : 0) >> 1;
#pragma unroll
    for (int r = 0; r < R; ++r) {
        const int rank = r * 64 + lane;
        if (rank < (int)p.cand_stride) {
            if (rank < kept) {
                p.cand[(size_t)qi * p.cand_stride + (kept - 1 - rank)] = L.lo[r] >> 1;
                if (p.cand_dist) p.cand_dist[(size_t)qi * p.cand_stride + (kept - 1 - rank)] = fkey_inv_out(L.hi[r], p.zero_dist_bits);
            } else {
                p.cand[(size_t)qi * p.cand_stride + rank] = kInvalidId;
                if (p.cand_dist) p.cand_dist[(size_t)qi * p.cand_stride + rank] = __builtin_inff();
            }
        }
    }
    if (lane == 0) {
        p.count[qi] = kept;
        p.hops[qi] = hops;
        p.dist_calc[qi] = dist_calc;
        atomicMax(p.max_dc, (uint32_t)dist_calc);
        if (p.edges) p.edges[qi] = edges;
        if (p.best) p.best[qi] = kth;
    }
}

template <int R>
__device__ __forceinline__ uint32_t reg_id_at_rank(const RegList<R>& L, int rank) {
    uint32_t v = (uint32_t)__shfl((int)(L.lo[0] >> 1), rank & 63);
#pragma unroll
    for (int r = 1; r < R; ++r) {
        const uint32_t t = (uint32_t)__shfl((int)(L.lo[r] >> 1), rank & 63);
        if ((rank >> 6) == r) v = t;
    }
    return v;
}


constexpr int kBigMaxEf = kRegListMaxEf;
#ifndef GBNNS_HOT2_MAX
#define GBNNS_HOT2_MAX 128
#endif
constexpr int kHot2MaxEf = GBNNS_HOT2_MAX;

__device__ __forceinline__ uint64_t dpp_wave_shl1_u64(uint64_t v) {
    const uint32_t lo = (uint32_t)__builtin_amdgcn_update_dpp(0, (int)(uint32_t)v, 0x130, 0xf, 0xf, false);
    const uint32_t hi = (uint32_t)__builtin_amdgcn_update_dpp(0, (int)(uint32_t)(v >> 32), 0x130, 0xf, 0xf, false);
    return ((uint64_t)hi << 32) | lo;
}

__host__ __device__ __forceinline__ constexpr bool big_list_flags_in_stage(int ef) {
    return (size_t)((ef + 63) / 64 * 64) + 64 <= (size_t)kRegStageSlots * 8;
}
__host__ __device__ __forceinline__ constexpr size_t big_list_fixed_bytes(int ef) {
    return (size_t)kRegTieCap * 8 + (size_t)kRegStageSlots * 8 + (size_t)((ef + 63) / 64 * 64) * 8 +
           (big_list_flags_in_stage(ef) ? 0 : (size_t)((ef + 63) / 64 * 64) + 64);
}

struct BigList {
    uint64_t* tie;
    uint64_t* stage;
    uint64_t* base;
    unsigned char* flags;
    RegList<1> F;
    int ef, l, f, tsize;
    uint32_t worst;
    uint32_t fworst;
    uint32_t mu_lo, mu_hi;
    bool c_valid;
    int p1, p2;
    uint32_t h1, n1, h2, n2;
#ifdef GBNNS_COOP_HINT
    uint32_t hint3;
#endif
#ifdef GBNNS_STAMPS
    unsigned long long st_flush = 0, st_refresh = 0, st_evict = 0;
    unsigned st_nflush = 0, st_nrefresh = 0, st_nbase = 0, st_nseq = 0, st_ninsert = 0, st_slow = 0;
#endif

    __device__ __forceinline__ void kill_front_from(int first_dead, int lane) {
        const bool dead = lane >= first_dead;
        F.lo[0] = dead ? 0xFFFFFFFFu : F.lo[0];
        F.hi[0] = dead ? 0xFFFFFFFFu : F.hi[0];
    }

    __device__ __forceinline__ uint64_t base_at(int rank) const {
        const uint64_t v = base[rank];
        return ((uint64_t)(uint32_t)__builtin_amdgcn_readfirstlane((int)(uint32_t)(v >> 32)) << 32) |
               (uint32_t)__builtin_amdgcn_readfirstlane((int)(uint32_t)v);
    }
    __device__ __forceinline__ uint32_t union_worst() const {
        const uint32_t lw = l > 0 ? (uint32_t)(base_at(l - 1) >> 32) : 0u;
        const uint32_t fw = f > 0 ? readlane_u32(F.hi[0], f - 1) : 0u;
        return lw > fw ? lw : fw;
    }
    __device__ __forceinline__ void trim_masks(int lane) {
        const int left = l - 64 * lane;
        const uint64_t keep = left >= 64 ? ~0ull : (left <= 0 ? 0ull : ((1ull << left) - 1ull));
        mu_lo &= (uint32_t)keep;
        mu_hi &= (uint32_t)(keep >> 32);
        if (p1 >= l || p2 >= l) c_valid = false;
    }
    __device__ __forceinline__ void refresh_cache(int lane) {
        STAMP(tr0)
#ifdef GBNNS_STAMPS
        st_nrefresh += 1;
#endif
        p1 = p2 = -1;
        h1 = h2 = 0xFFFFFFFFu;
        n1 = n2 = 0u;
        uint64_t nz = __ballot((mu_lo | mu_hi) != 0u);
        if (nz) {
            const int c1 = __ffsll((unsigned long long)nz) - 1;
            uint64_t m1 = ((uint64_t)readlane_u32(mu_hi, c1) << 32) | readlane_u32(mu_lo, c1);
            p1 = 64 * c1 + __ffsll((unsigned long long)m1) - 1;
            m1 &= m1 - 1;
            if (m1) {
                p2 = 64 * c1 + __ffsll((unsigned long long)m1) - 1;
            } else {
                nz &= nz - 1;
                if (nz) {
                    const int c2 = __ffsll((unsigned long long)nz) - 1;
                    const uint64_t m2 = ((uint64_t)readlane_u32(mu_hi, c2) << 32) | readlane_u32(mu_lo, c2);
                    p2 = 64 * c2 + __ffsll((unsigned long long)m2) - 1;
                }
            }
            const uint64_t kv = base[lane == 0 ? p1 : (p2 >= 0 ? p2 : p1)];
            h1 = readlane_u32((uint32_t)(kv >> 32), 0);
            n1 = readlane_u32((uint32_t)kv, 0) >> 1;
            if (p2 >= 0) {
                h2 = readlane_u32((uint32_t)(kv >> 32), 1);
                n2 = readlane_u32((uint32_t)kv, 1) >> 1;
            }
        }
        c_valid = true;
        STAMP(tr1)
#ifdef GBNNS_STAMPS
        st_refresh += tr1 - tr0;
#endif
    }
    __device__ __forceinline__ void expand_base(int p, int lane) {
        p = __builtin_amdgcn_readfirstlane(p);
#ifdef GBNNS_STAMPS
        st_nbase += 1;
#endif
        reinterpret_cast<uint32_t*>(base)[2 * p] |= 1u;
        const int c = p >> 6;
        uint64_t m = ((uint64_t)readlane_u32(mu_hi, c) << 32) | readlane_u32(mu_lo, c);
        m = clear_bit64(m, p & 63);
        mu_lo = writelane_u32(mu_lo, (uint32_t)m, c);
        mu_hi = writelane_u32(mu_hi, (uint32_t)(m >> 32), c);
        c_valid = false;
    }

    __device__ __forceinline__ void flush(int lane) {
        if (f == 0) return;
        STAMP(tf0)
        l = __builtin_amdgcn_readfirstlane(l);
        f = __builtin_amdgcn_readfirstlane(f);
        const int total = l + f;
        const int chunks = (total + 63) >> 6;
        {
            const int words = chunks * 8 + 8;
            for (int w0 = 0; w0 < words; w0 += 64)
                reinterpret_cast<uint64_t*>(flags)[w0 + lane < words ? w0 + lane : 0] = 0ull;
        }
        wave_sync();
        const uint64_t fk = ((uint64_t)F.hi[0] << 32) | F.lo[0];
        int lo = 0, hi = l;
        const int iters = 32 - __clz(l);
        for (int it = 0; it < iters; ++it) {
            const int mid = (lo + hi) >> 1;
            const uint64_t v = base[mid < l ? mid : 0];
            const bool go = lo < hi;
            const bool less = v < fk;
            lo = (go && less) ? mid + 1 : lo;
            hi = (go && !less) ? mid : hi;
        }
        flags[lane < f ? lo + lane : 64 * chunks + 1] = 1;
        wave_sync();
        uint32_t below = 0;
        {
            int carry = 0;
            for (int c = 0; c < chunks; ++c) {
                below = writelane_u32(below, (uint32_t)__builtin_amdgcn_readfirstlane(carry), c);
                carry += __popcll(__ballot(flags[64 * c + lane] != 0));
            }
        }
        mu_lo = mu_hi = 0u;
        for (int c = chunks - 1; c >= 0; --c) {
            const int rank = 64 * c + lane;
            const bool flagged = flags[rank] != 0;
            const uint64_t mk = __ballot(flagged);
            const int cc = (int)readlane_u32(below, c) +
                           (int)__builtin_amdgcn_mbcnt_hi((uint32_t)(mk >> 32), __builtin_amdgcn_mbcnt_lo((uint32_t)mk, 0u));
            const uint32_t flo = (uint32_t)__builtin_amdgcn_ds_bpermute((cc & 63) << 2, (int)F.lo[0]);
            const uint32_t fhi = (uint32_t)__builtin_amdgcn_ds_bpermute((cc & 63) << 2, (int)F.hi[0]);
            const int src = rank - cc;
            const uint64_t bv = (rank < total && src < l) ? base[src] : ~0ull;
            const uint64_t nk = flagged ? (((uint64_t)fhi << 32) | flo) : bv;
            base[rank] = nk;
            const uint64_t un = __ballot(rank < total && !((uint32_t)nk & 1u));
            mu_lo = writelane_u32(mu_lo, (uint32_t)un, c);
            mu_hi = writelane_u32(mu_hi, (uint32_t)(un >> 32), c);
        }
        wave_sync();
        l = total;
        f = 0;
        F.clear();
        c_valid = false;
        STAMP(tf1)
#ifdef GBNNS_STAMPS
        st_flush += tf1 - tf0;
        st_nflush += 1;
#endif
    }

    __device__ __forceinline__ bool offer_one(uint32_t dl, uint32_t nlo, int lane) {
        const bool full = l + f >= ef;
        if (full && !(dl < worst)) return true;
        if (f == 64) flush(lane);
        int ts_unused = 0;
        reg_offer<1>(dl, nlo, F, f, fworst, ts_unused, tie, 64, lane);
        if (!full) {
            if (l + f == ef) worst = union_worst();
            return true;
        }
        const uint64_t lt = l > 0 ? base_at(l - 1) : 0ull;
        const uint64_t ft = ((uint64_t)readlane_u32(F.hi[0], f - 1) << 32) | readlane_u32(F.lo[0], f - 1);
        uint64_t ev;
        if (lt > ft) {
            ev = lt;
            l -= 1;
            trim_masks(lane);
        } else {
            ev = ft;
            f -= 1;
            kill_front_from(f, lane);
        }
        const uint32_t nw = union_worst();
        if (nw != worst) {
            tsize = 0;
        } else if (!(ev & 1ull)) {
            if (tsize >= kRegTieCap) return false;
            tie[tsize] = ev;
            tsize += 1;
            wave_sync();
        }
        worst = nw;
        return true;
    }

    __device__ __forceinline__ bool insert(uint64_t m, uint32_t dk, uint32_t nb, int lane) {
        const int ns = __popcll(m);
        bool sequential = false;
        if (l + f + ns <= ef || (m & (m - 1)) != 0) {
            if (f + ns > 64) flush(lane);
            const uint32_t keep_lo = F.lo[0], keep_hi = F.hi[0], keep_fw = fworst;
            const int keep_f = f;
            int ts_unused = 0;
            if ((m & (m - 1)) != 0) {
                reg_merge(m, __builtin_amdgcn_inverse_ballot_w64(m), dk, nb, F, f, fworst, ts_unused, stage, 64, lane);
            } else {
                const int sl = __ffsll((unsigned long long)m) - 1;
                reg_offer<1>(readlane_u32(dk, sl), readlane_u32(nb, sl) << 1, F, f, fworst, ts_unused, tie, 64, lane);
            }
            const int E = l + f - ef;
            STAMP(te0)
            if (E > 0) {
                const int j = lane;
                const int bi = l - j;
                uint64_t H = base[(bi >= 0 && bi < l) ? bi : 0];
                H = bi < 0 ? 0ull : H;
                H = bi >= l ? ~0ull : H;
                const int fi = f - E - 1 + j;
                const uint32_t glo = (uint32_t)__builtin_amdgcn_ds_bpermute((fi & 63) << 2, (int)F.lo[0]);
                const uint32_t ghi = (uint32_t)__builtin_amdgcn_ds_bpermute((fi & 63) << 2, (int)F.hi[0]);
                uint64_t G = ((uint64_t)ghi << 32) | glo;
                G = fi < 0 ? 0ull : G;
                G = fi >= f ? ~0ull : G;
                const uint64_t La = H, Lb = dpp_wave_shl1_u64(H);
                const uint64_t Fb = G, Fa = dpp_wave_shl1_u64(G);
                const bool cand = j <= E && j <= l && E - j <= f;
                const uint64_t good = __ballot(cand && La > Fb && Fa > Lb);
                const int x = __ffsll((unsigned long long)good) - 1;
                const uint32_t la_hi = readlane_u32((uint32_t)(La >> 32), x), fa_hi = readlane_u32((uint32_t)(Fa >> 32), x);
                const uint32_t lb_hi = readlane_u32((uint32_t)(Lb >> 32), x), fb_hi = readlane_u32((uint32_t)(Fb >> 32), x);
                const uint32_t first_dropped = la_hi < fa_hi ? la_hi : fa_hi;
                const uint32_t nw = lb_hi > fb_hi ? lb_hi : fb_hi;
                if (first_dropped == nw) {
                    F.lo[0] = keep_lo; F.hi[0] = keep_hi; f = keep_f; fworst = keep_fw;
                    sequential = true;
                } else {
                    if (x > 0) {
                        l -= x;
                        trim_masks(lane);
                    }
                    f -= E - x;
                    kill_front_from(f, lane);
                    tsize = 0;
                    worst = nw;
                }
            } else if (E == 0) {
                worst = union_worst();
            }
            STAMP(te1)
#ifdef GBNNS_STAMPS
            st_evict += te1 - te0;
            st_ninsert += 1;
#endif
        } else {
            sequential = true;
        }
        if (sequential) {
#ifdef GBNNS_STAMPS
            st_nseq += 1;
#endif
            do {
                const int sl = __ffsll((unsigned long long)m) - 1;
                m &= m - 1;
                if (!offer_one(readlane_u32(dk, sl), readlane_u32(nb, sl) << 1, lane)) return false;
            } while (m);
        }
        return true;
    }

    __device__ __forceinline__ bool select(uint32_t& node, uint32_t& pred, uint32_t& h2k, int lane) {
        if (!c_valid) refresh_cache(lane);
        uint32_t ok, fb, q1, q2, hf1, hf2, nf1, nf2, hw, ha, na, hb, nb2, hr, t0;
        uint64_t fm;
#ifdef GBNNS_COOP_HINT
        uint32_t hint_;
#define GBNNS_SEL_HINT_LINE "s_cselect_b32 %[hint], %[nb2], %[na]\n\t"
#define GBNNS_SEL_HINT_OUT , [hint] "=&s"(hint_)
#else
#define GBNNS_SEL_HINT_LINE
#define GBNNS_SEL_HINT_OUT
#endif
        auto rfl = [](uint32_t v) { return (uint32_t)__builtin_amdgcn_readfirstlane((int)v); };
        asm volatile(
            "v_and_b32 %[t0], 1, %[flo]\n\t"
            "v_cmp_eq_u32 vcc, 0, %[t0]\n\t"
            "s_mov_b64 %[fm], vcc\n\t"
            "s_ff1_i32_b64 %[q1], %[fm]\n\t"
            "s_bitset0_b64 %[fm], %[q1]\n\t"
            "s_ff1_i32_b64 %[q2], %[fm]\n\t"
            "v_readlane_b32 %[hf1], %[fhi], %[q1]\n\t"
            "v_readlane_b32 %[nf1], %[flo], %[q1]\n\t"
            "v_readlane_b32 %[hf2], %[fhi], %[q2]\n\t"
            "v_readlane_b32 %[nf2], %[flo], %[q2]\n\t"
            "s_cmp_lt_i32 %[q1], 0\n\t"
            "s_cselect_b32 %[hf1], -1, %[hf1]\n\t"
            "s_cmp_lt_i32 %[q2], 0\n\t"
            "s_cselect_b32 %[hf2], -1, %[hf2]\n\t"
            "s_lshr_b32 %[nf1], %[nf1], 1\n\t"
            "s_lshr_b32 %[nf2], %[nf2], 1\n\t"
            "s_cmp_lt_u32 %[h1], %[hf1]\n\t"
            "s_cselect_b32 %[fb], 1, 0\n\t"
            "s_cselect_b32 %[hw], %[h1], %[hf1]\n\t"
            "s_cselect_b32 %[node], %[n1], %[nf1]\n\t"
            "s_cselect_b32 %[ha], %[h2], %[hf2]\n\t"
            "s_cselect_b32 %[na], %[n2], %[nf2]\n\t"
            "s_cselect_b32 %[hb], %[hf1], %[h1]\n\t"
            "s_cselect_b32 %[nb2], %[nf1], %[n1]\n\t"
            "s_min_u32 %[hr], %[ha], %[hb]\n\t"
            "s_cmp_lt_u32 %[ha], %[hb]\n\t"
            "s_cselect_b32 %[pred], %[na], %[nb2]\n\t"
            GBNNS_SEL_HINT_LINE
            "s_cmp_lg_u32 %[h1], %[hf1]\n\t"
            "s_cselect_b32 %[ok], 1, 0\n\t"
            "s_cmp_lg_u32 %[hr], %[hw]\n\t"
            "s_cselect_b32 %[ok], %[ok], 0\n\t"
            "s_cmp_eq_u32 %[ts], 0\n\t"
            "s_cselect_b32 %[ok], %[ok], 0\n\t"
            "s_cmp_lg_u32 %[ha], %[hb]\n\t"
            "s_cselect_b32 %[pred], %[pred], -1\n\t"
            "s_cselect_b32 %[hr], %[hr], -1\n\t"
            "s_cmp_lg_u32 %[hr], -1\n\t"
            "s_cselect_b32 %[pred], %[pred], -1"
            : [ok] "=&s"(ok), [fb] "=&s"(fb), [q1] "=&s"(q1), [q2] "=&s"(q2), [hf1] "=&s"(hf1), [hf2] "=&s"(hf2),
              [nf1] "=&s"(nf1), [nf2] "=&s"(nf2), [hw] "=&s"(hw), [ha] "=&s"(ha), [na] "=&s"(na), [hb] "=&s"(hb),
              [nb2] "=&s"(nb2), [hr] "=&s"(hr), [t0] "=&v"(t0), [fm] "=&s"(fm), [node] "=&s"(node), [pred] "=&s"(pred) GBNNS_SEL_HINT_OUT
            : [flo] "v"(F.lo[0]), [fhi] "v"(F.hi[0]), [h1] "s"(rfl(h1)), [n1] "s"(rfl(n1)), [h2] "s"(rfl(h2)), [n2] "s"(rfl(n2)), [ts] "s"(rfl((uint32_t)tsize))
            : "vcc", "scc");
        h2k = hr;
#ifdef GBNNS_COOP_HINT
        hint3 = hint_;
#endif
        if (__builtin_expect(ok != 0, 1)) {
            if (fb) expand_base(p1, lane);
            else F.lo[0] |= (lane == (int)q1) ? 1u : 0u;
            return true;
        }
        pred = kInvalidId;
        h2k = 0xFFFFFFFFu;
        const int pF = (int)q1;
        const uint32_t hF1 = hf1;
#ifdef GBNNS_STAMPS
        st_slow += 1;
#endif
        const bool any = p1 >= 0 || pF >= 0;
        const uint32_t hi_p = h1 < hF1 ? h1 : hF1;
        int bestL = -1, bestF = -1;
        uint32_t idL = 0, idF = 0;
        if (any) {
            if (p1 >= 0 && h1 == hi_p) {
                for (int b0 = p1; b0 < l; b0 += 64) {
                    const int r = b0 + lane;
                    uint64_t kv = base[r < l ? r : 0];
                    kv = r < l ? kv : ~0ull;
                    const bool same = (uint32_t)(kv >> 32) == hi_p;
                    const uint64_t ms = __ballot(same && !((uint32_t)kv & 1u));
                    if (ms) {
                        const int q = 63 - __clzll((long long)ms);
                        bestL = b0 + q;
                        idL = readlane_u32((uint32_t)kv, q) >> 1;
                    }
                    if (!((__ballot(same) >> 63) & 1ull)) break;
                }
            }
            const uint64_t msf = __ballot(!(F.lo[0] & 1u) && F.hi[0] == hi_p);
            if (msf) {
                bestF = 63 - __clzll((long long)msf);
                idF = readlane_u32(F.lo[0], bestF) >> 1;
            }
        }
        const bool pickL = bestL >= 0 && (bestF < 0 || idL > idF);
        const bool have = bestL >= 0 || bestF >= 0;
        const uint32_t lid = pickL ? idL : idF;
        if (tsize > 0 && (!have || hi_p == worst)) {
            uint32_t v = (lane < tsize) ? key_id(tie[lane]) + 1u : 0u;
            int w = lane;
#pragma unroll
            for (int off = 32; off > 0; off >>= 1) {
                const uint32_t ov = (uint32_t)__shfl_xor((int)v, off);
                const int ow = __shfl_xor(w, off);
                if (ov > v) { v = ov; w = ow; }
            }
            v = (uint32_t)__builtin_amdgcn_readfirstlane((int)v);
            w = __builtin_amdgcn_readfirstlane(w);
            if (!have || v - 1u > lid) {
                node = v - 1u;
                tie[w] = tie[tsize - 1];
                tsize -= 1;
                wave_sync();
                return true;
            }
        }
        if (!have) return false;
        node = lid;
        if (pickL) expand_base(bestL, lane);
        else F.lo[0] |= (lane == bestF) ? 1u : 0u;
        return true;
    }
    template <int DEEP = 8>
    __device__ __forceinline__ void finish(const WalkParams& p, uint32_t qi, int hops, int dist_calc, int edges,
                                           unsigned char* rr_scratch, int lane) {
        flush(lane);
        const int kept = l < p.k ? l : p.k;
        for (int rank = lane; rank < (int)p.cand_stride; rank += 64) {
            const uint64_t kv = base[rank < kept ? rank : 0];
            const size_t at = (size_t)qi * p.cand_stride + (rank < kept ? kept - 1 - rank : rank);
            p.cand[at] = rank < kept ? key_id(kv) : kInvalidId;
            if (p.cand_dist) p.cand_dist[at] = rank < kept ? fkey_inv_out(key_hi(kv), p.zero_dist_bits) : __builtin_inff();
        }
        if (lane == 0) {
            p.count[qi] = kept;
            p.hops[qi] = hops;
            p.dist_calc[qi] = dist_calc;
            atomicMax(p.max_dc, (uint32_t)dist_calc);
            if (p.edges) p.edges[qi] = edges;
            if (p.best) p.best[qi] = kept > 0 ? key_id(base[kept - 1]) : kInvalidId;
        }
        if (p.rr_db) {
            const uint64_t* b = base;
            fused_rerank<DEEP>(p, qi, kept, rr_scratch, lane, [&](int rank) { return key_id(b[rank]); });
        }
    }

    __device__ __forceinline__ void init(unsigned char* smem, int ef_) {
        const int ef_pad = (ef_ + 63) & ~63;
        tie = reinterpret_cast<uint64_t*>(smem);
        stage = tie + kRegTieCap;
        base = stage + kRegStageSlots;
        flags = big_list_flags_in_stage(ef_) ? reinterpret_cast<unsigned char*>(stage) : reinterpret_cast<unsigned char*>(base + ef_pad);
        F.clear();
        ef = ef_; l = 0; f = 1; tsize = 0;
        mu_lo = mu_hi = 0u;
        c_valid = false; p1 = p2 = -1; h1 = h2 = 0xFFFFFFFFu; n1 = n2 = 0u;
        worst = fworst = 0u;
    }
};
}

}
```

Baseline: 32.47 million.

## Add block markers and hop counters; fuse DPP adds and tweak merge rank loop

Inserts assembly label markers into a custom section and optional hop-count instrumentation throughout the walk kernel. It also fuses the DPP move plus packed add into v_add_f32_dpp in the distance reductions and uses m0 directly in the merge rank loop, saving an SGPR and an s_mov per iteration. The distance macros gain a W0 wait parameter in place of the fixed vmcnt(3), and the selection paths reorder some min/prefetch logic. The instrumentation is off by default, while the marker labels are always emitted but add no instructions.

```diff
diff --git a/gbnns_dim_red_amd/csrc/walk_hot.hip b/gbnns_dim_red_amd/csrc/walk_hot.hip
--- a/gbnns_dim_red_amd/csrc/walk_hot.hip
+++ b/gbnns_dim_red_amd/csrc/walk_hot.hip
@@ -17,6 +17,48 @@
         hi_p = readlane_u32(L.hi[0], __ffsll((unsigned long long)mu) - 1);
         const uint64_t ms = __ballot(!(L.lo[0] & 1u) && L.hi[0] == hi_p) & lmask;
         if (ms) best = 63 - __clzll((long long)ms);
+    }
+    if (tsize > 0 && (best < 0 || hi_p == worst)) {
+        uint32_t v = (lane < tsize) ? key_id(tie[lane]) + 1u : 0u;
+        int w = lane;
+        int lane_here = lane;
+        asm volatile(GBNNS_MARK_STR(GBNNS_BLK_SEL_SLOW) : "+v"(lane_here));
+#pragma unroll
+        for (int off = 32; off > 0; off >>= 1) {
+            const int partner = (lane_here ^ off) << 2;
+            const uint32_t ov = (uint32_t)__builtin_amdgcn_ds_bpermute(partner, (int)v);
+            const int ow = __builtin_amdgcn_ds_bpermute(partner, w);
+            if (ov > v) { v = ov; w = ow; }
+        }
+        v = (uint32_t)__builtin_amdgcn_readfirstlane((int)v);
+        w = __builtin_amdgcn_readfirstlane(w);
+        const uint32_t lid = (best >= 0) ? (readlane_u32(L.lo[0], best) >> 1) : 0u;
+        if (best < 0 || v - 1u > lid) {
+            node = v - 1u;
+            if (lane == 0) tie[w] = tie[tsize - 1];
+            tsize -= 1;
+            wave_sync();
+            return true;
+        }
+    }
+    if (best < 0) return false;
+    node = readlane_u32(L.lo[0], best) >> 1;
+    if (lane == best) L.lo[0] |= 1u;
+    return true;
+}
+
+template <int R>
+__device__ __forceinline__ bool regN_select_slow(RegList<R>& L, int p1, int& tsize, uint64_t* tie, uint32_t worst, int ef,
+                                                 int lane, uint32_t& node) {
+    int best = -1;
+    uint32_t hi_p = 0;
+    if (p1 >= 0) {
+        hi_p = L.hi_at(p1);
+#pragma unroll
+        for (int r = 0; r < R; ++r) {
+            const uint64_t ms = __ballot(!(L.lo[r] & 1u) && L.hi[r] == hi_p) & RegList<R>::lane_mask(r, ef);
+            if (ms) best = r * 64 + 63 - __clzll((long long)ms);
+        }
     }
     if (tsize > 0 && (best < 0 || hi_p == worst)) {
         uint32_t v = (lane < tsize) ? key_id(tie[lane]) + 1u : 0u;
@@ -32,48 +74,6 @@
         }
         v = (uint32_t)__builtin_amdgcn_readfirstlane((int)v);
         w = __builtin_amdgcn_readfirstlane(w);
-        const uint32_t lid = (best >= 0) ? (readlane_u32(L.lo[0], best) >> 1) : 0u;
-        if (best < 0 || v - 1u > lid) {
-            node = v - 1u;
-            if (lane == 0) tie[w] = tie[tsize - 1];
-            tsize -= 1;
-            wave_sync();
-            return true;
-        }
-    }
-    if (best < 0) return false;
-    node = readlane_u32(L.lo[0], best) >> 1;
-    if (lane == best) L.lo[0] |= 1u;
-    return true;
-}
-
-template <int R>
-__device__ __forceinline__ bool regN_select_slow(RegList<R>& L, int p1, int& tsize, uint64_t* tie, uint32_t worst, int ef,
-                                                 int lane, uint32_t& node) {
-    int best = -1;
-    uint32_t hi_p = 0;
-    if (p1 >= 0) {
-        hi_p = L.hi_at(p1);
-#pragma unroll
-        for (int r = 0; r < R; ++r) {
-            const uint64_t ms = __ballot(!(L.lo[r] & 1u) && L.hi[r] == hi_p) & RegList<R>::lane_mask(r, ef);
-            if (ms) best = r * 64 + 63 - __clzll((long long)ms);
-        }
-    }
-    if (tsize > 0 && (best < 0 || hi_p == worst)) {
-        uint32_t v = (lane < tsize) ? key_id(tie[lane]) + 1u : 0u;
-        int w = lane;
-        int lane_here = lane;
-        asm volatile("" : "+v"(lane_here));
-#pragma unroll
-        for (int off = 32; off > 0; off >>= 1) {
-            const int partner = (lane_here ^ off) << 2;
-            const uint32_t ov = (uint32_t)__builtin_amdgcn_ds_bpermute(partner, (int)v);
-            const int ow = __builtin_amdgcn_ds_bpermute(partner, w);
-            if (ov > v) { v = ov; w = ow; }
-        }
-        v = (uint32_t)__builtin_amdgcn_readfirstlane((int)v);
-        w = __builtin_amdgcn_readfirstlane(w);
         const uint32_t lid = (best >= 0) ? (L.lo_at(best) >> 1) : 0u;
         if (best < 0 || v - 1u > lid) {
             node = v - 1u;
@@ -90,6 +90,7 @@
 }
 
 #define GBNNS_VS_ASM(T0, T1, T2, ADDR)                                                                                                   \
+        GBNNS_MARK_STR(GBNNS_BLK_VS_HASH)                                                                              \
         "s_bfe_u32 %[mulc], %[shr], 0x50008\n\t"                                    \
         "s_lshl_b32 %[mulc], 0x9E3779B1, %[mulc]\n\t"                                                                  \
         "v_mul_lo_u32 " T0 ", %[id], %[mulc]\n\t"                                                                       \
@@ -99,8 +100,9 @@
         "s_cmp_lg_u32 %[shr], 0\n\t"                                                                                   \
         "v_mul_hi_u32 " T1 ", " T0 ", %[nb]\n\t"                                                                         \
         "v_lshl_add_u32 " ADDR ", " T1 ", 4, %[basev]\n\t"                                                               \
-        "s_cbranch_scc1 4f\n"                                                                                          \
-        "1:\n\t"                                                                                                       \
+        "s_cbranch_scc1 4f\n\t"                                                                                       \
+        GBNNS_MARK_STR(GBNNS_BLK_VS_PACKED)                                                                            \
+        "\n1:\n\t"                                                                                                     \
         "ds_read_b128 v[60:63], " ADDR "\n\t"                                                                           \
         "s_waitcnt lgkmcnt(0)\n\t"                                                                                     \
         "v_bfe_u32 v56, v60, 0, 24\n\t"                                                                    \
@@ -147,11 +149,13 @@
         "v_cndmask_b32 " ADDR ", " ADDR ", %[basev], vcc\n\t"                                                            \
         "s_branch 1b\n"                                                                                                \
         "4:\n\t"                                                                          \
+        GBNNS_MARK_STR(GBNNS_BLK_VS_Q_KEY)                                                                             \
         "s_lshl_b32 %[mulc], %[nb], 4\n\t"                                                                             \
         "v_mul_lo_u32 " T0 ", " T0 ", %[nb]\n\t"                               \
         "v_lshrrev_b32 " T0 ", %[shr], " T0 "\n\t"                                                           \
         "v_lshl_or_b32 " T2 ", " T0 ", 16, " T0 "\n"                          \
         "5:\n\t"                                                                                                       \
+        GBNNS_MARK_STR(GBNNS_BLK_VS_Q_TEST) GBNNS_HOPC_ASM("cq")                                                       \
         "ds_read_b128 v[60:63], " ADDR "\n\t"                                                                           \
         "s_waitcnt lgkmcnt(0)\n\t"                                                                                     \
         "v_xor_b32 v56, v60, " T2 "\n\t"                                                                                \
@@ -166,6 +170,7 @@
         "v_cmp_ne_u32 vcc, 0, v56\n\t"                                                                                 \
         "s_and_b64 exec, exec, vcc\n\t"                                                                                \
         "s_cbranch_execz 9f\n\t"                                                                                       \
+        GBNNS_MARK_STR(GBNNS_BLK_VS_Q_CLAIM) GBNNS_HOPC_ASM("cc")                                                      \
         "s_mov_b64 %[act], exec\n\t"                                                                                   \
         "v_cmp_gt_u32 vcc, 7, " T1 "\n\t"                                                                               \
         "s_and_b64 exec, exec, vcc\n\t"                                                                                \
@@ -184,6 +189,7 @@
         "6:\n\t"                                                                                                       \
         "s_mov_b64 exec, %[act]\n\t"                                                                                   \
         "s_cbranch_execz 9f\n\t"                                                                                       \
+        GBNNS_MARK_STR(GBNNS_BLK_VS_Q_NEXT) GBNNS_HOPC_ASM("cn")                                                       \
         "v_and_b32 " T0 ", 7, " T2 "\n\t"                         \
         "v_lshl_add_u32 " T0 ", " T0 ", 4, 16\n\t"                \
         "v_add_u32 " ADDR ", " ADDR ", " T0 "\n\t"                                                                        \
@@ -202,8 +208,9 @@
         "s_cbranch_execnz 5b\n"                                                                                        \
         "9:\n\t"
 
-#define GBNNS_L2_DIST_ASM(Q0A, Q0B, Q1A, Q1B, Q2A, Q2B, Q3A, Q3B, W1, W2, W3)                                                     \
-        "s_waitcnt vmcnt(3)\n\t"                                \
+#define GBNNS_L2_DIST_ASM(Q0A, Q0B, Q1A, Q1B, Q2A, Q2B, Q3A, Q3B, W0, W1, W2, W3)                                                 \
+        GBNNS_MARK_STR(GBNNS_BLK_DIST)                                                                                 \
+        W0                                                      \
         "v_pk_add_f32 v[40:41], v[40:41], " Q0A " neg_lo:[0,1] neg_hi:[0,1]\n\t"                                        \
         "v_pk_add_f32 v[42:43], v[42:43], " Q0B " neg_lo:[0,1] neg_hi:[0,1]\n\t"                                        \
         "v_pk_mul_f32 v[40:41], v[40:41], v[40:41]\n\t"                                                                \
@@ -229,13 +236,11 @@
         "v_pk_add_f32 v[62:63], v[62:63], v[50:51]\n\t"                                                                \
         "v_pk_add_f32 v[60:61], v[60:61], v[52:53]\n\t"                                                                \
         "v_pk_add_f32 v[62:63], v[62:63], v[54:55]\n\t"                                                                \
-        "s_nop 1\n\t"                                                                                                  \
-        "v_mov_b32_dpp v56, v60 quad_perm:[0,0,2,2] row_mask:0xf bank_mask:0xf\n\t"                                    \
-        "v_mov_b32_dpp v57, v61 quad_perm:[0,0,2,2] row_mask:0xf bank_mask:0xf\n\t"                                    \
-        "v_mov_b32_dpp v58, v62 quad_perm:[0,0,2,2] row_mask:0xf bank_mask:0xf\n\t"                                    \
-        "v_mov_b32_dpp v59, v63 quad_perm:[0,0,2,2] row_mask:0xf bank_mask:0xf\n\t"                                    \
-        "v_pk_add_f32 v[56:57], v[56:57], v[40:41]\n\t"                               \
-        "v_pk_add_f32 v[58:59], v[58:59], v[42:43]\n\t"                                                                \
+        "s_nop 1\n\t"                                         \
+        "v_add_f32_dpp v56, v60, v40 quad_perm:[0,0,2,2] row_mask:0xf bank_mask:0xf\n\t"    \
+        "v_add_f32_dpp v57, v61, v41 quad_perm:[0,0,2,2] row_mask:0xf bank_mask:0xf\n\t"    \
+        "v_add_f32_dpp v58, v62, v42 quad_perm:[0,0,2,2] row_mask:0xf bank_mask:0xf\n\t"    \
+        "v_add_f32_dpp v59, v63, v43 quad_perm:[0,0,2,2] row_mask:0xf bank_mask:0xf\n\t"    \
         "v_pk_add_f32 v[56:57], v[56:57], v[44:45]\n\t"                                                                \
         "v_pk_add_f32 v[58:59], v[58:59], v[46:47]\n\t"                                                                \
         "v_pk_add_f32 v[56:57], v[56:57], v[48:49]\n\t"                                                                \
@@ -247,8 +252,9 @@
         "v_add_f32 %[key], %[key], v59\n\t"                                                                            \
         "v_or_b32 %[key], 0x80000000, %[key]"
 
-#define GBNNS_DOT_DIST_ASM(Q0A, Q0B, Q1A, Q1B, Q2A, Q2B, Q3A, Q3B, W1, W2, W3)                                                    \
-        "s_waitcnt vmcnt(3)\n\t"                                                                                       \
+#define GBNNS_DOT_DIST_ASM(Q0A, Q0B, Q1A, Q1B, Q2A, Q2B, Q3A, Q3B, W0, W1, W2, W3)                                                \
+        GBNNS_MARK_STR(GBNNS_BLK_DIST)                                                                                 \
+        W0                                                                                                             \
         "v_pk_mul_f32 v[40:41], v[40:41], " Q0A "\n\t"                                                                 \
         "v_pk_mul_f32 v[42:43], v[42:43], " Q0B "\n\t"                                                                 \
         W1                                                                                                             \
@@ -270,13 +276,11 @@
         "v_pk_add_f32 v[62:63], v[62:63], v[50:51]\n\t"                                                                \
         "v_pk_add_f32 v[60:61], v[60:61], v[52:53]\n\t"                                                                \
         "v_pk_add_f32 v[62:63], v[62:63], v[54:55]\n\t"                                                                \
-        "s_nop 1\n\t"                                                                                                  \
-        "v_mov_b32_dpp v56, v60 quad_perm:[0,0,2,2] row_mask:0xf bank_mask:0xf\n\t"      \
-        "v_mov_b32_dpp v57, v61 quad_perm:[0,0,2,2] row_mask:0xf bank_mask:0xf\n\t"                                    \
-        "v_mov_b32_dpp v58, v62 quad_perm:[0,0,2,2] row_mask:0xf bank_mask:0xf\n\t"                                    \
-        "v_mov_b32_dpp v59, v63 quad_perm:[0,0,2,2] row_mask:0xf bank_mask:0xf\n\t"                                    \
-        "v_pk_add_f32 v[56:57], v[60:61], v[56:57]\n\t"                             \
-        "v_pk_add_f32 v[58:59], v[62:63], v[58:59]\n\t"                                                                \
+        "s_nop 1\n\t"                                         \
+        "v_add_f32_dpp v56, v60, v60 quad_perm:[0,0,2,2] row_mask:0xf bank_mask:0xf\n\t"                               \
+        "v_add_f32_dpp v57, v61, v61 quad_perm:[0,0,2,2] row_mask:0xf bank_mask:0xf\n\t"                               \
+        "v_add_f32_dpp v58, v62, v62 quad_perm:[0,0,2,2] row_mask:0xf bank_mask:0xf\n\t"                               \
+        "v_add_f32_dpp v59, v63, v63 quad_perm:[0,0,2,2] row_mask:0xf bank_mask:0xf\n\t"                               \
         "v_add_f32 %[key], v56, v57\n\t"                                                    \
         "v_add_f32 v60, v58, v59\n\t"                                               \
         "v_add_f32 %[key], %[key], v60\n\t"                                                                            \
@@ -314,7 +318,7 @@
         "10:\n\t"                               \
         GBNNS_LOADS_TESTED(O1, O2, O3)          \
         "11:\n\t"
-#define GBNNS_HOT_END "\n8:\n\ts_mov_b64 exec, %[sv]"
+#define GBNNS_HOT_END "\n8:\n\ts_mov_b64 exec, %[sv]\n\t" GBNNS_MARK_STR(GBNNS_BLK_MASK)
 
 #define GBNNS_HOT_CLOBBERS_40                                                                                           \
     "vcc", "scc", "memory", "v40", "v41", "v42", "v43", "v44", "v45", "v46", "v47", "v48", "v49", "v50", "v51", "v52", "v53", "v54",  \
@@ -323,12 +327,20 @@
 template <int METRIC = 0, bool QLDS = false, bool SPEC = !QLDS, bool DYN = false, typename QP>
 __device__ __forceinline__ uint32_t hot_expand(const char* db_base, uint32_t roff, uint32_t nb, uint64_t valid, uint32_t lds_base,
                                                uint32_t nbuckets, QP qh, uint32_t qaddr, uint64_t& claimed, uint32_t shr, uint64_t& overflowed,
-                                               uint32_t spec = 0u) {
+                                               uint32_t spec = 0u, unsigned* hopc = nullptr) {
     const uint32_t end = lds_base + (nbuckets << 4);
     uint32_t basev = lds_base, key, mulc;
     uint64_t fresh, act, sv;
+#ifdef GBNNS_HOP_COUNTS
+    unsigned hopc_none[3] = {0, 0, 0};
+    unsigned* const hc = hopc ? hopc + 8 : hopc_none;
+    unsigned cq = hc[0], cc = hc[1], cn = hc[2];
+#define GBNNS_HOPC_OUT , [cq] "+s"(cq), [cc] "+s"(cc), [cn] "+s"(cn)
+#else
+#define GBNNS_HOPC_OUT
+#endif
 #define GBNNS_Q(T) [qa##T] "v"(f32x2{qh[T].x, qh[T].y}), [qb##T] "v"(f32x2{qh[T].z, qh[T].w})
-#define GBNNS_HOT_OUT [fresh] "=&s"(fresh), [act] "=&s"(act), [sv] "=&s"(sv), [mulc] "=&s"(mulc), [key] "=&v"(key)
+#define GBNNS_HOT_OUT [fresh] "=&s"(fresh), [act] "=&s"(act), [sv] "=&s"(sv), [mulc] "=&s"(mulc), [key] "=&v"(key) GBNNS_HOPC_OUT
 #define GBNNS_HOT_IN [id] "v"(nb), [valid] "s"(valid), [end] "s"(end), [basev] "v"(basev), [shr] "s"(shr), [nb] "s"(nbuckets), \
                      [roff] "v"(roff), [db] "s"(db_base)
 #define GBNNS_HOT_IN_QREG GBNNS_HOT_IN, GBNNS_Q(0), GBNNS_Q(1), GBNNS_Q(2), GBNNS_Q(3)
@@ -342,31 +354,32 @@
 #define GBNNS_CLOB_QLDS "v36", "v37", "v38", "v39", GBNNS_HOT_CLOBBERS_40
 #define GBNNS_HOT_STMT(LOADS_BEFORE, VS, AFTER_VS, DIST, OUTS, OPS, CLOB)                      \
     asm volatile("s_mov_b64 %[sv], exec\n\t"                                                   \
-                 "s_mov_b64 exec, %[valid]\n\t" LOADS_BEFORE VS AFTER_VS DIST GBNNS_HOT_END      \
+                 "s_mov_b64 exec, %[valid]\n\t" GBNNS_MARK_STR(GBNNS_BLK_LOADS_SPEC) LOADS_BEFORE VS \
+                 GBNNS_MARK_STR(GBNNS_BLK_LOADS) AFTER_VS GBNNS_MARK_STR(GBNNS_BLK_QPIECES) DIST GBNNS_HOT_END \
                  : OUTS                                                                        \
                  : OPS                                                                         \
                  : CLOB)
 #define GBNNS_RESTORE_EXEC "s_mov_b64 exec, %[sv]\n\t"
 #define GBNNS_L2_QREG                                                                                                          \
-    GBNNS_L2_DIST_ASM("%[qa0]", "%[qb0]", "%[qa1]", "%[qb1]", "%[qa2]", "%[qb2]", "%[qa3]", "%[qb3]", "s_waitcnt vmcnt(2)\n\t", \
+    GBNNS_L2_DIST_ASM("%[qa0]", "%[qb0]", "%[qa1]", "%[qb1]", "%[qa2]", "%[qb2]", "%[qa3]", "%[qb3]", "s_waitcnt vmcnt(3)\n\t", "s_waitcnt vmcnt(2)\n\t", \
                       "s_waitcnt vmcnt(1)\n\t", "s_waitcnt vmcnt(0)\n\t")
 #define GBNNS_L2_QLDS                                                                                                          \
     "ds_read_b128 v[36:39], %[qaddr]\n\t"                       \
     "ds_read_b128 v[56:59], %[qaddr] offset:16\n\t"           \
     "ds_read_b128 v[60:63], %[qaddr] offset:32\n\t"                                                                           \
-    "s_waitcnt lgkmcnt(2)\n\t"                                                                                                \
     GBNNS_L2_DIST_ASM("v[36:37]", "v[38:39]", "v[56:57]", "v[58:59]", "v[60:61]", "v[62:63]", "v[36:37]", "v[38:39]",          \
+                      "s_waitcnt vmcnt(3) lgkmcnt(2)\n\t",      \
                       "ds_read_b128 v[36:39], %[qaddr] offset:48\n\ts_waitcnt vmcnt(2) lgkmcnt(2)\n\t",                        \
                       "s_waitcnt vmcnt(1) lgkmcnt(1)\n\t", "s_waitcnt vmcnt(0) lgkmcnt(0)\n\t")
 #define GBNNS_DOT_QREG                                                                                                          \
-    GBNNS_DOT_DIST_ASM("%[qa0]", "%[qb0]", "%[qa1]", "%[qb1]", "%[qa2]", "%[qb2]", "%[qa3]", "%[qb3]", "s_waitcnt vmcnt(2)\n\t", \
+    GBNNS_DOT_DIST_ASM("%[qa0]", "%[qb0]", "%[qa1]", "%[qb1]", "%[qa2]", "%[qb2]", "%[qa3]", "%[qb3]", "s_waitcnt vmcnt(3)\n\t", "s_waitcnt vmcnt(2)\n\t", \
                        "s_waitcnt vmcnt(1)\n\t", "s_waitcnt vmcnt(0)\n\t")
 #define GBNNS_DOT_QLDS                                                                                                         \
     "ds_read_b128 v[36:39], %[qaddr]\n\t"                                                                                     \
     "ds_read_b128 v[56:59], %[qaddr] offset:32\n\t"                                                                           \
     "ds_read_b128 v[60:63], %[qaddr] offset:64\n\t"                                                                           \
-    "s_waitcnt lgkmcnt(2)\n\t"                                                                                                \
     GBNNS_DOT_DIST_ASM("v[36:37]", "v[38:39]", "v[56:57]", "v[58:59]", "v[60:61]", "v[62:63]", "v[36:37]", "v[38:39]",         \
+                       "s_waitcnt vmcnt(3) lgkmcnt(2)\n\t",                                                                   \
                        "ds_read_b128 v[36:39], %[qaddr] offset:96\n\ts_waitcnt vmcnt(2) lgkmcnt(2)\n\t",                       \
                        "s_waitcnt vmcnt(1) lgkmcnt(1)\n\t", "s_waitcnt vmcnt(0) lgkmcnt(0)\n\t")
     uint32_t t0, t1, t2, addr;
@@ -399,6 +412,10 @@
 #undef GBNNS_Q
 #undef GBNNS_HOT_OUT
 #undef GBNNS_HOT_IN
+#undef GBNNS_HOPC_OUT
+#ifdef GBNNS_HOP_COUNTS
+    hc[0] = cq; hc[1] = cc; hc[2] = cn;
+#endif
     claimed = fresh & 0x5555555555555555ull;
     overflowed = fresh & 0xAAAAAAAAAAAAAAAAull;
     return key;
@@ -470,13 +487,22 @@
 #ifdef GBNNS_LIFE_STAMPS
     const unsigned long long life1 = __builtin_amdgcn_s_memrealtime();
 #endif
+#ifdef GBNNS_HOP_COUNTS
+    unsigned hopc[32];
+#pragma unroll
+    for (int i = 0; i < 32; ++i) hopc[i] = 0;
+#else
+    unsigned* const hopc = nullptr;
+#endif
 
     while (true) {
         uint32_t node, pred, ok, h2;
+        HOPC(0, 1);
         if constexpr (R == 1) {
             uint64_t fm;
             uint32_t t0, q1, q2, h1;
             asm volatile(
+                GBNNS_MARK_STR(GBNNS_BLK_SEL)
                 "v_and_b32 %[t0], 1, %[lo]\n\t"
                 "v_cmp_eq_u32 vcc, 0, %[t0]\n\t"
                 "s_and_b64 %[fm], vcc, %[lmask]\n\t"
@@ -491,24 +517,24 @@
                 "v_readlane_b32 %[pred], %[lo], %[q2]\n\t"
                 "s_lshr_b32 %[node], %[node], 1\n\t"
                 "s_lshr_b32 %[pred], %[pred], 1\n\t"
+                "s_cmp_lt_i32 %[q2], 0\n\t"
+                "s_cselect_b32 %[pred], -1, %[pred]\n\t"
+                "s_cselect_b32 %[h2], -1, %[h2]\n\t"
                 "s_cmp_lg_u32 %[h1], %[h2]\n\t"
                 "s_cselect_b32 %[ok], 1, 0\n\t"
-                "s_cmp_lt_i32 %[q2], 0\n\t"
-                "s_cselect_b32 %[ok], 1, %[ok]\n\t"
-                "s_cselect_b32 %[pred], -1, %[pred]\n\t"
-                "s_cselect_b32 %[h2], -1, %[h2]\n\t"
                 "s_cmp_lt_i32 %[q1], 0\n\t"
                 "s_cselect_b32 %[ok], 0, %[ok]\n\t"
                 "s_cmp_lg_u32 %[ok], 0\n\t"
                 "s_cselect_b32 %[q1], %[q1], -1\n\t"
                 "v_cmp_eq_u32 vcc, %[q1], %[lane]\n\t"
-                "v_cndmask_b32 %[t0], 0, 1, vcc\n\t"
-                "v_or_b32 %[lo], %[lo], %[t0]"
+                "v_addc_co_u32 %[lo], vcc, 0, %[lo], vcc\n\t"
+                GBNNS_MARK_STR(GBNNS_BLK_ADJ)
                 : [lo] "+v"(L.lo[0]), [fm] "=&s"(fm), [t0] "=&v"(t0), [q1] "=&s"(q1), [q2] "=&s"(q2), [h1] "=&s"(h1),
                   [h2] "=&s"(h2), [node] "=&s"(node), [pred] "=&s"(pred), [ok] "=&s"(ok)
                 : [hi] "v"(L.hi[0]), [lmask] "s"(lmask), [tsize] "s"(tsize), [lane] "v"(lane)
                 : "vcc", "scc");
             if (__builtin_expect(ok == 0, 0)) {
+                HOPC(1, 1);
                 const uint64_t mu = __ballot(!(L.lo[0] & 1u)) & lmask;
                 if (!reg1_select_slow(L, mu, tsize, tie, worst, lmask, lane, node)) break;
                 pred = kInvalidId;
@@ -547,14 +573,18 @@
             }
         }
 
+        hops += 1;
         uint32_t nb, nbw = kInvalidId;
         if (node == pf_node) {
+            HOPC(3, 1);
             nb = pf_val;
             if constexpr (WIDE) nbw = pf_valw;
         } else if (node == pf2_node) {
+            HOPC(4, 1);
             nb = pf2_val;
             if constexpr (WIDE) nbw = pf2_valw;
         } else {
+            HOPC(2, 1);
             nb = *reinterpret_cast<const uint32_t*>(ell_base + node * ell_row_bytes + slot_off);
             if constexpr (WIDE) nbw = *reinterpret_cast<const uint32_t*>(ell_base + node * ell_row_bytes + slotw_off);
         }
@@ -565,6 +595,7 @@
         const uint64_t mv1 = WIDE ? __ballot(nbw != kInvalidId) : 0ull;
         pf_node = pred;
         if (pred != kInvalidId) {
+            HOPC(5, 1);
             pf_val = *reinterpret_cast<const uint32_t*>(ell_base + pred * ell_row_bytes + slot_off);
             if constexpr (WIDE) pf_valw = *reinterpret_cast<const uint32_t*>(ell_base + pred * ell_row_bytes + slotw_off);
         }
@@ -572,18 +603,27 @@
             if (__builtin_expect(mv == 0, 0)) return true;
             if (__builtin_expect((uint32_t)dist_calc > dc_limit, 0)) return false;
             edges += __popcll(mv & 0x5555555555555555ull);
+            HOPC(6, 1);
+            HOPC(7, spec_tail);
             uint64_t mclaimed, movf;
-            const uint32_t kd = hot_expand<METRIC, QLDS, SPEC, (QLDS && !SPEC)>(db_base, (nb << 7) + half * (METRIC == 0 ? 64u : 16u), nb, mv, hash_lds, nbuckets, qreg.v, qaddr, mclaimed, vs_shr, movf, spec_tail);
+            const uint32_t kd = hot_expand<METRIC, QLDS, SPEC, (QLDS && !SPEC)>(db_base, (nb << 7) + half * (METRIC == 0 ? 64u : 16u), nb, mv, hash_lds, nbuckets, qreg.v, qaddr, mclaimed, vs_shr, movf, spec_tail, hopc);
+            HOPC(11, (mclaimed | movf) != 0);
             if (__builtin_expect(movf != 0, 0)) {
+                GBNNS_MARK(GBNNS_BLK_STASH);
+                HOPC(23, 1);
                 if (!stash_claim(hash_lds, nbuckets, movf >> 1, nb, mclaimed, lane)) return false;
             }
             const uint64_t mfresh = mclaimed << 1;
             const uint32_t dk = __builtin_amdgcn_inverse_ballot_w64(mfresh) ? kd : 0xFFFFFFFFu;
             dist_calc += __popcll(mfresh);
+            HOPC(12, __popcll(mfresh));
             uint64_t m = size < ef ? mfresh : __ballot(dk < worst);
             if (m != 0) {
+                HOPC(13, 1);
+                HOPC(14, __popcll(m));
                 auto prefetch2 = [&](const uint32_t dmin, const uint64_t me) {
-                    if (dmin < h2 && me != 0 && (me & (me - 1)) == 0) {
+                    if (me != 0 && (me & (me - 1)) == 0) {
+                        HOPC(18, 1);
                         pf2_node = readlane_u32(nb, __ffsll((unsigned long long)me) - 1);
                         pf2_val = *reinterpret_cast<const uint32_t*>(ell_base + pf2_node * ell_row_bytes + slot_off);
                         if constexpr (WIDE) {
@@ -598,23 +638,58 @@
                         merged = reg_merge_cb<true>(m, __builtin_amdgcn_inverse_ballot_w64(m), dk, nb, L, size, worst, tsize, stage, ef, lane,
                                                     [&](const uint32_t dmin) { if (dmin < h2) prefetch2(dmin, __ballot(dk == dmin) & m); });
                     } else {
-                        prefetch2(readlane_u32(dk, __ffsll((unsigned long long)m) - 1), m);
+                        const uint32_t d1 = readlane_u32(dk, __ffsll((unsigned long long)m) - 1);
+                        if (d1 < h2) prefetch2(d1, m);
                     }
                 } else {
-                    uint32_t x = dk;
-                    x = min(x, (uint32_t)__builtin_amdgcn_update_dpp((int)x, (int)x, 0xB1, 0xf, 0xf, false));
-                    x = min(x, (uint32_t)__builtin_amdgcn_update_dpp((int)x, (int)x, 0x4E, 0xf, 0xf, false));
-                    x = min(x, (uint32_t)__builtin_amdgcn_update_dpp((int)x, (int)x, 0x141, 0xf, 0xf, false));
-                    x = min(x, (uint32_t)__builtin_amdgcn_update_dpp((int)x, (int)x, 0x140, 0xf, 0xf, false));
-                    const uint32_t dmin = min(min(readlane_u32(x, 0), readlane_u32(x, 16)), min(readlane_u32(x, 32), readlane_u32(x, 48)));
-                    if (dmin < h2) prefetch2(dmin, __ballot(dk == dmin) & m);
-                    if ((m & (m - 1)) != 0) {
+                    const uint64_t mc = R == 1 ? __ballot(dk < h2) & m : 0ull;
+                    if constexpr (R != 1) {
+                        uint32_t x = dk;
+                        x = min(x, (uint32_t)__builtin_amdgcn_update_dpp((int)x, (int)x, 0xB1, 0xf, 0xf, false));
+                        x = min(x, (uint32_t)__builtin_amdgcn_update_dpp((int)x, (int)x, 0x4E, 0xf, 0xf, false));
+                        x = min(x, (uint32_t)__builtin_amdgcn_update_dpp((int)x, (int)x, 0x141, 0xf, 0xf, false));
+                        x = min(x, (uint32_t)__builtin_amdgcn_update_dpp((int)x, (int)x, 0x140, 0xf, 0xf, false));
+                        const uint32_t dmin = min(min(readlane_u32(x, 0), readlane_u32(x, 16)), min(readlane_u32(x, 32), readlane_u32(x, 48)));
+                        if (dmin < h2) prefetch2(dmin, __ballot(dk == dmin) & m);
+                    } else if (mc != 0) {
+                        uint64_t me = mc;
+                        uint32_t dmin = 0u;
+                        int nc;
+                        asm("s_bcnt1_i32_b64 %0, %1" : "=s"(nc) : "s"(mc) : "scc");
+                        if (nc > 1) {
+                            HOPC(16, 1);
+                            HOPC(17, nc);
+                            uint32_t x;
+                            asm volatile("s_nop 1\n\t"
+                                         "v_min_u32_dpp %0, %1, %1 quad_perm:[2,3,0,1] row_mask:0xf bank_mask:0xf\n\t"
+                                         "s_nop 1\n\t"
+                                         "v_min_u32_dpp %0, %0, %0 row_ror:4 row_mask:0xf bank_mask:0xf\n\t"
+                                         "s_nop 1\n\t"
+                                         "v_min_u32_dpp %0, %0, %0 row_ror:8 row_mask:0xf bank_mask:0xf"
+                                         : "=&v"(x) : "v"(dk));
+                            dmin = min(min(readlane_u32(x, 1), readlane_u32(x, 17)), min(readlane_u32(x, 33), readlane_u32(x, 49)));
+                            me = __ballot(dk == dmin) & mc;
+                        } else {
+                            HOPC(15, 1);
+                            if constexpr (WIDE) dmin = readlane_u32(dk, __ffsll((unsigned long long)mc) - 1);
+                        }
+                        prefetch2(dmin, me);
+                    }
+                    int ns;
+                    if constexpr (R == 1) asm("s_bcnt1_i32_b64 %0, %1" : "=s"(ns) : "s"(m) : "scc");
+                    else ns = (m & (m - 1)) != 0 ? 2 : 1;
+                    if (ns > 1) {
+                        HOPC(19, 1);
+                        HOPC(20, __popcll(m));
                         if constexpr (R == 1) merged = reg_merge(m, __builtin_amdgcn_inverse_ballot_w64(m), dk, nb, L, size, worst, tsize, stage, ef, lane);
                         else merged = reg_merge_multi<R>(m, __builtin_amdgcn_inverse_ballot_w64(m), dk, nb, L, size, worst, tsize, stage, ef, lane);
+                        HOPC(21, !merged);
                     }
                 }
                 if (!merged) {
+                    GBNNS_MARK(GBNNS_BLK_SEQ);
                     do {
+                        HOPC(22, 1);
                         const int l = __ffsll((unsigned long long)m) - 1;
                         m &= m - 1;
                         if (!reg_offer<R>(readlane_u32(dk, l), readlane_u32(nb, l) << 1, L, size, worst, tsize, tie, ef, lane)) return false;
@@ -627,8 +702,16 @@
         if constexpr (WIDE) {
             if (!expand_pass(nbw, mv1)) { handed_over = true; break; }
         }
-        hops += 1;
-    }
+    }
+    GBNNS_MARK(GBNNS_BLK_EPILOGUE);
+#ifdef GBNNS_HOP_COUNTS
+    hopc[24] = 1;
+    hopc[25] = handed_over ? 0u : (unsigned)hops;
+    if (lane == 0 && p.stamps) {
+#pragma unroll
+        for (int i = 0; i < 32; ++i) atomicAdd(p.stamps + i, (unsigned long long)hopc[i]);
+    }
+#endif
 
     if (handed_over) {
         if (lane == 0) {
diff --git a/gbnns_dim_red_amd/csrc/walk_lists.h b/gbnns_dim_red_amd/csrc/walk_lists.h
--- a/gbnns_dim_red_amd/csrc/walk_lists.h
+++ b/gbnns_dim_red_amd/csrc/walk_lists.h
@@ -37,6 +37,42 @@
 __device__ __forceinline__ uint32_t readlane_u32(uint32_t v, int l) {
     return (uint32_t)__builtin_amdgcn_readlane((int)v, l);
 }
+
+#define GBNNS_MARK_STR2(ID) ".Lgbm%=_" #ID ":\n\t.pushsection .gbnns_marks,\"\",@progbits\n\t.quad .Lgbm%=_" #ID "\n\t.quad " #ID "\n\t.popsection\n\t"
+#define GBNNS_MARK_STR(ID) GBNNS_MARK_STR2(ID)
+#ifdef GBNNS_NO_CXX_MARKS
+#define GBNNS_MARK(ID)
+#else
+#define GBNNS_MARK(ID) asm volatile(GBNNS_MARK_STR(ID) ::)
+#endif
+#define GBNNS_BLK_SEL 1
+#define GBNNS_BLK_SEL_SLOW 2
+#define GBNNS_BLK_ADJ 3
+#define GBNNS_BLK_LOADS_SPEC 5
+#define GBNNS_BLK_VS_HASH 6
+#define GBNNS_BLK_VS_PACKED 7
+#define GBNNS_BLK_VS_Q_KEY 8
+#define GBNNS_BLK_VS_Q_TEST 9
+#define GBNNS_BLK_VS_Q_CLAIM 10
+#define GBNNS_BLK_VS_Q_NEXT 11
+#define GBNNS_BLK_LOADS 12
+#define GBNNS_BLK_QPIECES 13
+#define GBNNS_BLK_DIST 14
+#define GBNNS_BLK_MASK 15
+#define GBNNS_BLK_STASH 16
+#define GBNNS_BLK_RANK_HEAD 18
+#define GBNNS_BLK_RANK 19
+#define GBNNS_BLK_SCATTER 20
+#define GBNNS_BLK_SEQ 21
+#define GBNNS_BLK_EPILOGUE 23
+
+#ifdef GBNNS_HOP_COUNTS
+#define HOPC(i, v) hopc[i] += (unsigned)(v)
+#define GBNNS_HOPC_ASM(NAME) "s_add_u32 %[" NAME "], %[" NAME "], 1\n\t"
+#else
+#define HOPC(i, v)
+#define GBNNS_HOPC_ASM(NAME)
+#endif
 
 #ifdef GBNNS_STAMPS
 #define STAMP(var)                                                                        \
@@ -363,19 +399,20 @@
     const uint32_t slo = nb << 1;
     const uint64_t skey = ((uint64_t)dk << 32) | slo;
     const bool is_entry = lane < size;
-    uint32_t shift, rank, below, sl_, t_, smin = 0xFFFFFFFFu;
+    uint32_t shift, rank, below, t_, smin = 0xFFFFFFFFu;
     uint64_t ma, mb, mm = m;
 #define GBNNS_RANK_LOOP(MIN_STEP)                                                                                       \
     asm volatile(                                                                                                      \
+        GBNNS_MARK_STR(GBNNS_BLK_RANK_HEAD)                                                                            \
         "v_mov_b32 %[shift], 0\n\t"                                                                                    \
         "v_mov_b32 %[rank], 0\n\t"                                                                                     \
         "v_mov_b32 %[below], 0\n"                                                                                      \
         "1:\n\t"                                                                                                       \
-        "s_ff1_i32_b64 %[sl], %[mm]\n\t"                                                                               \
-        "v_readlane_b32 " GBNNS_MERGE_SHI ", %[dk], %[sl]\n\t"                                                                         \
-        "v_readlane_b32 " GBNNS_MERGE_SLO ", %[slo], %[sl]\n\t"                                                                        \
-        "s_bitset0_b64 %[mm], %[sl]\n\t"                                                                               \
-        "s_mov_b32 m0, %[sl]\n\t"                                                                                      \
+        GBNNS_MARK_STR(GBNNS_BLK_RANK)                                                                                 \
+        "s_ff1_i32_b64 m0, %[mm]\n\t"                           \
+        "v_readlane_b32 " GBNNS_MERGE_SHI ", %[dk], m0\n\t"                                                                            \
+        "v_readlane_b32 " GBNNS_MERGE_SLO ", %[slo], m0\n\t"                                                                           \
+        "s_bitset0_b64 %[mm], m0\n\t"                                                                                  \
         "v_cmp_gt_u64_e64 %[ma], %[key], " GBNNS_MERGE_SPAIR "\n\t"                                                                 \
         "v_cmp_gt_u64_e64 %[mb], %[skey], " GBNNS_MERGE_SPAIR "\n\t" MIN_STEP                                                       \
         "s_bcnt0_i32_b64 %[t], %[ma]\n\t"                                                                              \
@@ -383,8 +420,9 @@
         "v_addc_co_u32_e64 %[rank], vcc, 0, %[rank], %[mb]\n\t"                                                        \
         "v_writelane_b32 %[below], %[t], m0\n\t"                                                                       \
         "s_cmp_lg_u64 %[mm], 0\n\t"                                                                                    \
-        "s_cbranch_scc1 1b"                                                                                            \
-        : [shift] "=&v"(shift), [rank] "=&v"(rank), [below] "=&v"(below), [sl] "=&s"(sl_), [t] "=&s"(t_), [ma] "=&s"(ma), \
+        "s_cbranch_scc1 1b\n\t"                                                                                        \
+        GBNNS_MARK_STR(GBNNS_BLK_SCATTER)                                                                              \
+        : [shift] "=&v"(shift), [rank] "=&v"(rank), [below] "=&v"(below), [t] "=&s"(t_), [ma] "=&s"(ma),                  \
           [mb] "=&s"(mb), [mm] "+s"(mm), [smin] "+s"(smin)                                                              \
         : [dk] "v"(dk), [slo] "v"(slo), [key] "v"(key), [skey] "v"(skey)                                                \
         : "vcc", "scc", "m0", GBNNS_MERGE_SLO, GBNNS_MERGE_SHI)
```

Result: no change. 32.61 million (median of 2 runs) (+0.5%).
